# AlonKellner/hifi-gan

Measured on NVIDIA B200. Metric: V1 audio samples/sec, higher is better.
Workload: dtype bf16

## Files before the change

hifi-gan_b200/_lib.py:

```python
from __future__ import annotations

import ctypes
import hashlib
import os
import shutil
import subprocess
import threading
import time
from ctypes import POINTER, byref, c_char_p, c_double, c_float, c_int, c_int64, c_void_p

_HERE = os.path.dirname(os.path.abspath(__file__))
CSRC = os.path.join(_HERE, "csrc")
LIB_PATH = os.path.join(_HERE, "libhifigan_b200.so")
SOURCES = ["hg_api.cu", "hg_conv1d_tc.cu", "hg_resblock_pair.cu", "hg_disc.cu", "hg_prep.cu", "hg_mel.cu",
           "hg_wgrad.cu", "hg_train.cu", "hg_batched.cu"]
NVCC_FLAGS = ["-gencode", "arch=compute_100a,code=sm_100a", "-O3", "-lineinfo", "-std=c++17",
              "-Xcompiler", "-fPIC", "-shared"]

_lock = threading.Lock()
_lib = None


class HgError(RuntimeError):
    pass


HASH_PATH = os.path.join(_HERE, "libhifigan_b200.srchash")
_LOCK_PATH = os.path.join(_HERE, ".build.lock")


def _source_hash() -> str:
    h = hashlib.sha256(" ".join(NVCC_FLAGS).encode())
    deps = sorted(os.path.join(CSRC, f) for f in os.listdir(CSRC) if f.endswith((".cu", ".cuh", ".h")))
    deps.append(os.path.join(os.path.dirname(_HERE), "include", "hifigan_b200.h"))
    for d in deps:
        if os.path.isfile(d):
            h.update(os.path.basename(d).encode())
            with open(d, "rb") as f:
                h.update(f.read())
    return h.hexdigest()


def _stale() -> bool:
    if not os.path.exists(LIB_PATH) or not os.path.exists(HASH_PATH):
        return True
    with open(HASH_PATH) as f:
        return f.read().strip() != _source_hash()


def build(force: bool = False, verbose: bool = False) -> str:
    if not force and not _stale():
        return LIB_PATH
    nvcc = shutil.which("nvcc") or "/usr/local/cuda/bin/nvcc"
    if not os.path.exists(nvcc):
        raise HgError("nvcc not found: cannot build libhifigan_b200.so")
    deadline = time.time() + 900
    while True:
        try:
            fd = os.open(_LOCK_PATH, os.O_CREAT | os.O_EXCL | os.O_WRONLY)
            os.close(fd)
            break
        except FileExistsError:
            if time.time() > deadline or time.time() - os.path.getmtime(_LOCK_PATH) > 900:
                try:
                    os.unlink(_LOCK_PATH)
                except FileNotFoundError:
                    pass
            time.sleep(0.5)
    try:
        if not force and not _stale():
            return LIB_PATH
        tmp = LIB_PATH + f".tmp{os.getpid()}"
        cmd = [nvcc] + NVCC_FLAGS + ["-o", tmp] + [os.path.join(CSRC, s) for s in SOURCES]
        if verbose:
            cmd.insert(1, "-Xptxas=-v")
        res = subprocess.run(cmd, capture_output=True, text=True)
        if res.returncode != 0:
            if os.path.exists(tmp):
                os.unlink(tmp)
            raise HgError("nvcc failed:\n" + res.stdout + res.stderr)
        if verbose:
            print(res.stderr)
        os.replace(tmp, LIB_PATH)
        with open(HASH_PATH + ".tmp", "w") as f:
            f.write(_source_hash())
        os.replace(HASH_PATH + ".tmp", HASH_PATH)
    finally:
        try:
            os.unlink(_LOCK_PATH)
        except FileNotFoundError:
            pass
    return LIB_PATH


_SIGNATURES = {
    "hg_version": (c_char_p, []),
    "hg_last_error": (c_char_p, []),
    "hg_abi_version": (c_int, []),
    "hg_launch_count": (c_int64, []),
    "hg_timestamp": (c_int, [c_void_p, c_void_p]),
    "hg_pack_conv1d_weight": (c_int, [c_void_p, c_void_p, c_int, c_int, c_int, c_int, c_void_p, c_void_p]),
    "hg_convtr1d_geometry": (c_int, [c_int, c_int, c_int, POINTER(c_int), POINTER(c_int)]),
    "hg_pack_convtr1d_weight": (c_int, [c_void_p, c_void_p, c_int, c_int, c_int, c_int, c_int, c_void_p, c_void_p]),
    "hg_conv1d_fwd": (c_int, [c_void_p, c_void_p, c_void_p, c_int, c_int, c_int, c_int, c_int, c_int, c_int,
                              c_void_p, c_void_p, c_void_p, c_float, c_void_p, c_void_p, c_float, c_void_p, c_int,
                              c_void_p]),
    "hg_conv1d_tap_order": (c_int, [c_int, c_int, c_int, POINTER(c_int)]),
    "hg_conv1d_general_fwd": (c_int, [c_void_p, c_void_p, c_void_p, c_int, c_int, c_int, c_int, c_int, c_int, c_int,
                                      c_int, c_int, c_int, c_void_p, c_float, c_void_p, c_int, c_int, c_void_p]),
    "hg_disc_first_conv_fwd": (c_int, [c_void_p, c_void_p, c_void_p, c_int, c_int, c_int, c_int, c_int, c_int, c_int,
                                       c_int, c_void_p, c_float, c_void_p]),
    "hg_disc_last_conv_fwd": (c_int, [c_void_p, c_void_p, c_void_p, c_int, c_int, c_int, c_int, c_int, c_void_p,
                                      c_void_p]),
    "hg_avgpool_4_2_2_fwd": (c_int, [c_void_p, c_int, c_int, c_void_p, c_void_p]),
    "hg_disc_export_fmap": (c_int, [c_void_p, c_int, c_int, c_int, c_int, c_int, c_void_p, c_void_p]),
    "hg_disc_import_fmap": (c_int, [c_void_p, c_int, c_int, c_int, c_int, c_int, c_void_p, c_void_p]),
    "hg_prep_job_size": (c_int, []),
    "hg_prep_batched": (c_int, [c_void_p, c_void_p, c_int, c_int, c_int, c_void_p]),
    "hg_resblock_pair_supported": (c_int, [c_int, c_int, c_int]),
    "hg_resblock_single_supported": (c_int, [c_int, c_int, c_int]),
    "hg_resblock_pair_fwd": (c_int, [c_void_p, c_void_p, c_void_p, c_void_p, c_void_p, c_int, c_int, c_int, c_int,
                                     c_int, c_float, c_void_p, c_void_p, c_float, c_void_p, c_void_p, c_float,
                                     c_void_p, c_int, c_void_p]),
    "hg_float_to_int16": (c_int, [c_void_p, ctypes.c_longlong, c_float, c_void_p, c_void_p]),
    "hg_loss_sum": (c_int, [c_void_p, c_void_p, ctypes.c_longlong, c_int, c_float, c_void_p, c_void_p]),
    "hg_segment_gather": (c_int, [c_void_p, c_void_p, c_void_p, c_int, c_int, c_void_p, c_void_p]),
    "hg_ncl_to_nlc": (c_int, [c_void_p, c_int, c_int, c_int, c_int, c_void_p, c_void_p, c_float, c_void_p]),
    "hg_nlc_to_ncl": (c_int, [c_void_p, c_int, c_int, c_int, c_void_p, c_void_p]),
    "hg_conv_post_tanh_fwd": (c_int, [c_void_p, c_void_p, c_void_p, c_int, c_int, c_int, c_int, c_void_p, c_void_p]),
    "hg_mel_plan_create": (c_int, [POINTER(c_void_p), c_int, c_int, c_int, c_int, c_int, c_double, c_double, c_void_p]),
    "hg_mel_plan_destroy": (c_int, [c_void_p]),
    "hg_mel_num_frames": (c_int, [c_void_p, c_int]),
    "hg_mel_fwd": (c_int, [c_void_p, c_void_p, c_int, c_int, c_void_p, c_void_p, c_void_p]),
    "hg_mel_bwd": (c_int, [c_void_p, c_void_p, c_void_p, c_int, c_int, c_void_p, c_void_p]),
    "hg_mel_emulate_host": (c_int, [c_void_p, c_void_p, c_int, c_int, c_void_p]),
    "hg_mel_bwd_emulate_host": (c_int, [c_void_p, c_void_p, c_void_p, c_int, c_int, c_void_p]),
    "hg_pack_dgrad_weight": (c_int, [c_void_p, c_int, c_int, c_int, c_void_p, c_void_p]),
    "hg_conv1d_dgrad": (c_int, [c_void_p, c_void_p] + [c_int] * 12 + [c_void_p, c_float, c_void_p, c_void_p, c_float,
                                c_void_p, c_void_p, c_void_p, c_float, c_void_p, c_int, c_int, c_int, c_int,
                                c_void_p, c_void_p, c_void_p, c_void_p, c_int, c_void_p]),
    "hg_conv1d_wgrad": (c_int, [c_void_p, c_void_p] + [c_int] * 11 + [c_void_p, c_int, c_void_p]),
    "hg_unpack_wgrad_conv": (c_int, [c_void_p] + [c_int] * 7 + [POINTER(c_int), c_void_p, c_void_p]),
    "hg_wgrad_finish_conv": (c_int, [c_void_p] + [c_int] * 7 + [POINTER(c_int), c_void_p, c_void_p, c_int, c_void_p,
                                                                  c_void_p, c_void_p]),
    "hg_wgrad_finish_convtr": (c_int, [c_void_p] + [c_int] * 7 + [c_void_p, c_void_p, c_int, c_void_p, c_void_p,
                                                                    c_void_p]),
    "hg_weight_norm_bwd": (c_int, [c_void_p, c_void_p, c_void_p, c_int, c_int, c_int, c_void_p, c_void_p, c_void_p]),
    "hg_fold_weight_norm": (c_int, [c_void_p, c_void_p, c_int, c_int, c_void_p, c_void_p]),
    "hg_pack_disc_weight": (c_int, [c_void_p] + [c_int] * 7 + [c_void_p, c_void_p, c_void_p]),
    "hg_spectral_norm_fwd": (c_int, [c_void_p, c_void_p, c_void_p, c_int, c_int, c_int, c_void_p, c_void_p, c_void_p,
                                     c_void_p, c_void_p, c_void_p]),
    "hg_spectral_norm_bwd": (c_int, [c_void_p, c_void_p, c_void_p, c_void_p, c_void_p, c_int, c_int, c_int, c_void_p,
                                     c_void_p, c_void_p]),
    "hg_colsum_bf16": (c_int, [c_void_p, c_int, c_int, c_int, c_int, c_int, c_void_p, c_void_p]),
    "hg_conv_post_tanh_bwd": (c_int, [c_void_p, c_void_p, c_void_p, c_void_p, c_int, c_int, c_int, c_int, c_float,
                                      c_float, c_void_p, c_void_p, c_void_p, c_void_p, c_void_p, c_void_p, c_void_p,
                                      c_void_p]),
    "hg_disc_last_conv_bwd": (c_int, [c_void_p, c_void_p, c_void_p, c_int, c_int, c_int, c_int, c_int, c_float,
                                      c_void_p, c_float, c_void_p, c_void_p, c_void_p, c_void_p, c_void_p, c_void_p]),
    "hg_disc_first_conv_bwd": (c_int, [c_void_p, c_void_p, c_void_p] + [c_int] * 8 + [c_void_p] * 4),
    "hg_avgpool_4_2_2_bwd": (c_int, [c_void_p, c_int, c_int, c_void_p, c_void_p]),
    "hg_loss_grad": (c_int, [c_void_p, c_void_p, ctypes.c_longlong, c_int, c_float, c_float, c_float, c_void_p,
                             c_void_p, c_void_p]),
    "hg_adamw_step": (c_int, [c_void_p, c_void_p, c_void_p, c_void_p, ctypes.c_longlong, c_float, c_float, c_float,
                              c_float, c_float, c_int, c_void_p, c_void_p, c_float, c_void_p]),
}

EXPORTED_SYMBOLS = tuple(_SIGNATURES)


def lib() -> ctypes.CDLL:
    global _lib
    if _lib is not None:
        return _lib
    with _lock:
        if _lib is None:
            if _stale():
                build()
            handle = ctypes.CDLL(LIB_PATH)
            for name, (res, args) in _SIGNATURES.items():
                fn = getattr(handle, name)
                fn.restype = res
                fn.argtypes = args
            if handle.hg_abi_version() != 3:
                raise HgError("libhifigan_b200.so ABI mismatch")
            _lib = handle
    return _lib


def check(rc: int, what: str = "") -> None:
    if rc != 0:
        msg = lib().hg_last_error().decode("utf-8", "replace")
        raise HgError(f"{what or 'hifigan_b200'} failed (code {rc}): {msg}")


def launch_count() -> int:
    return int(lib().hg_launch_count())
```

hifi-gan_b200/csrc/hg_common.cuh:

```cuda
#pragma once

#include <cuda_runtime.h>
#include <cuda_bf16.h>
#include <cuda.h>
#include <stdint.h>
#include <stdio.h>

#define HG_OK 0
#define HG_ERR_INVALID (-1)
#define HG_ERR_CUDA (-2)
#define HG_ERR_UNSUPPORTED (-3)
#define HG_ERR_DRIVER (-4)

void hg_set_error(const char* fmt, ...);

#define HG_CHECK_CUDA(expr)                                                        \
  do {                                                                             \
    cudaError_t _e = (expr);                                                       \
    if (_e != cudaSuccess) {                                                       \
      hg_set_error("%s:%d: %s -> %s", __FILE__, __LINE__, #expr,                   \
                   cudaGetErrorString(_e));                                        \
      return HG_ERR_CUDA;                                                          \
    }                                                                              \
  } while (0)

#define HG_REQUIRE(cond, ...)                                                      \
  do {                                                                             \
    if (!(cond)) {                                                                 \
      hg_set_error(__VA_ARGS__);                                                   \
      return HG_ERR_INVALID;                                                       \
    }                                                                              \
  } while (0)

namespace hg {

#ifndef HG_SPIN_LIMIT
#define HG_SPIN_LIMIT (1u << 28)
#endif

__device__ __forceinline__ uint32_t smem_u32(const void* p) {
  return static_cast<uint32_t>(__cvta_generic_to_shared(p));
}

__device__ __forceinline__ bool elect_one() {
  uint32_t pred = 0;
  asm volatile(
      "{\n\t"
      ".reg .pred P;\n\t"
      "elect.sync _|P, 0xffffffff;\n\t"
      "selp.b32 %0, 1, 0, P;\n\t"
      "}\n"
      : "=r"(pred));
  return pred != 0;
}

__device__ __forceinline__ void mbar_init(uint64_t* bar, uint32_t count) {
  asm volatile("mbarrier.init.shared::cta.b64 [%0], %1;" ::"r"(smem_u32(bar)), "r"(count));
}
__device__ __forceinline__ void fence_mbar_init() {
  asm volatile("fence.mbarrier_init.release.cluster;" ::: "memory");
}
__device__ __forceinline__ void fence_proxy_async_smem() {
  asm volatile("fence.proxy.async.shared::cta;" ::: "memory");
}
__device__ __forceinline__ void mbar_arrive(uint64_t* bar) {
  asm volatile("mbarrier.arrive.shared::cta.b64 _, [%0];" ::"r"(smem_u32(bar)) : "memory");
}
__device__ __forceinline__ void mbar_arrive_expect_tx(uint64_t* bar, uint32_t bytes) {
  asm volatile("mbarrier.arrive.expect_tx.shared::cta.b64 _, [%0], %1;" ::"r"(smem_u32(bar)),
               "r"(bytes)
               : "memory");
}
__device__ __forceinline__ bool mbar_try_wait(uint64_t* bar, uint32_t parity) {
  uint32_t ok;
  asm volatile(
      "{\n\t"
      ".reg .pred P;\n\t"
      "mbarrier.try_wait.parity.shared::cta.b64 P, [%1], %2;\n\t"
      "selp.b32 %0, 1, 0, P;\n\t"
      "}\n"
      : "=r"(ok)
      : "r"(smem_u32(bar)), "r"(parity)
      : "memory");
  return ok != 0;
}
__device__ __forceinline__ void mbar_wait(uint64_t* bar, uint32_t parity) {
  uint32_t spins = 0;
  while (!mbar_try_wait(bar, parity)) {
    if (++spins > HG_SPIN_LIMIT) {
      printf("hg: mbarrier wait timed out (block %d thread %d)\n", (int)blockIdx.x, (int)threadIdx.x);
      __trap();
    }
  }
}

__device__ __forceinline__ void tma_prefetch_desc(const CUtensorMap* m) {
  asm volatile("prefetch.tensormap [%0];" ::"l"(reinterpret_cast<uint64_t>(m)) : "memory");
}
__device__ __forceinline__ void tma_load_3d(void* smem_dst, const CUtensorMap* m, uint64_t* bar,
                                            int32_t c0, int32_t c1, int32_t c2) {
  asm volatile(
      "cp.async.bulk.tensor.3d.shared::cluster.global.mbarrier::complete_tx::bytes"
      " [%0], [%1, {%3, %4, %5}], [%2];"
      :
      : "r"(smem_u32(smem_dst)), "l"(reinterpret_cast<uint64_t>(m)), "r"(smem_u32(bar)), "r"(c0),
        "r"(c1), "r"(c2)
      : "memory");
}

__device__ __forceinline__ void tc_fence_before() {
  asm volatile("tcgen05.fence::before_thread_sync;" ::: "memory");
}
__device__ __forceinline__ void tc_fence_after() {
  asm volatile("tcgen05.fence::after_thread_sync;" ::: "memory");
}
__device__ __forceinline__ void tmem_alloc(uint32_t* smem_result, uint32_t ncols) {
  asm volatile("tcgen05.alloc.cta_group::1.sync.aligned.shared::cta.b32 [%0], %1;" ::"r"(
                   smem_u32(smem_result)),
               "r"(ncols)
               : "memory");
  asm volatile("tcgen05.relinquish_alloc_permit.cta_group::1.sync.aligned;" ::: "memory");
}
__device__ __forceinline__ void tmem_dealloc(uint32_t taddr, uint32_t ncols) {
  asm volatile("tcgen05.dealloc.cta_group::1.sync.aligned.b32 %0, %1;" ::"r"(taddr), "r"(ncols)
               : "memory");
}
__device__ __forceinline__ void umma_bf16_ss_lo(uint32_t d_tmem, uint32_t a_lo, uint32_t b_lo,
                                                uint32_t desc_hi, uint32_t idesc, uint32_t accumulate) {
  asm volatile(
      "{\n\t"
      ".reg .pred p;\n\t"
      ".reg .b64 da, db;\n\t"
      "setp.ne.b32 p, %5, 0;\n\t"
      "mov.b64 da, {%1, %3};\n\t"
      "mov.b64 db, {%2, %3};\n\t"
      "tcgen05.mma.cta_group::1.kind::f16 [%0], da, db, %4, p;\n\t"
      "}\n"
      :
      : "r"(d_tmem), "r"(a_lo), "r"(b_lo), "r"(desc_hi), "r"(idesc), "r"(accumulate)
      : "memory");
}
__device__ __forceinline__ uint32_t cluster_ctarank() {
  uint32_t r;
  asm volatile("mov.u32 %0, %%cluster_ctarank;" : "=r"(r));
  return r;
}
__device__ __forceinline__ void cluster_sync_all() {
  asm volatile("barrier.cluster.arrive.release.aligned;" ::: "memory");
  asm volatile("barrier.cluster.wait.acquire.aligned;" ::: "memory");
}
__device__ __forceinline__ void mbar_arrive_remote(uint64_t* bar, uint32_t cta) {
  asm volatile(
      "{\n\t"
      ".reg .b32 remAddr32;\n\t"
      "mapa.shared::cluster.u32 remAddr32, %0, %1;\n\t"
      "mbarrier.arrive.shared::cluster.b64 _, [remAddr32];\n\t"
      "}\n"
      :
      : "r"(smem_u32(bar)), "r"(cta)
      : "memory");
}
__device__ __forceinline__ void tma_load_3d_2sm(void* smem_dst, const CUtensorMap* m, uint64_t* bar,
                                                int32_t c0, int32_t c1, int32_t c2) {
  asm volatile(
      "cp.async.bulk.tensor.3d.cta_group::2.shared::cluster.global.mbarrier::complete_tx::bytes"
      " [%0], [%1, {%3, %4, %5}], [%2];"
      :
      : "r"(smem_u32(smem_dst)), "l"(reinterpret_cast<uint64_t>(m)), "r"(smem_u32(bar) & 0xFEFFFFFFu),
        "r"(c0), "r"(c1), "r"(c2)
      : "memory");
}
__device__ __forceinline__ void tmem_alloc_2sm(uint32_t* smem_result, uint32_t ncols) {
  asm volatile("tcgen05.alloc.cta_group::2.sync.aligned.shared::cta.b32 [%0], %1;" ::"r"(
                   smem_u32(smem_result)),
               "r"(ncols)
               : "memory");
  asm volatile("tcgen05.relinquish_alloc_permit.cta_group::2.sync.aligned;" ::: "memory");
}
__device__ __forceinline__ void tmem_dealloc_2sm(uint32_t taddr, uint32_t ncols) {
  asm volatile("tcgen05.dealloc.cta_group::2.sync.aligned.b32 %0, %1;" ::"r"(taddr), "r"(ncols)
               : "memory");
}
__device__ __forceinline__ void umma_bf16_ss_lo_2sm(uint32_t d_tmem, uint32_t a_lo, uint32_t b_lo,
                                                    uint32_t desc_hi, uint32_t idesc, uint32_t accumulate) {
  asm volatile(
      "{\n\t"
      ".reg .pred p;\n\t"
      ".reg .b64 da, db;\n\t"
      "setp.ne.b32 p, %5, 0;\n\t"
      "mov.b64 da, {%1, %3};\n\t"
      "mov.b64 db, {%2, %3};\n\t"
      "tcgen05.mma.cta_group::2.kind::f16 [%0], da, db, %4, p;\n\t"
      "}\n"
      :
      : "r"(d_tmem), "r"(a_lo), "r"(b_lo), "r"(desc_hi), "r"(idesc), "r"(accumulate)
      : "memory");
}
__device__ __forceinline__ void umma_commit_2sm(uint64_t* bar) {
  asm volatile(
      "tcgen05.commit.cta_group::2.mbarrier::arrive::one.shared::cluster.multicast::cluster.b64 [%0], %1;"
      :
      : "r"(smem_u32(bar)), "h"(static_cast<uint16_t>(3))
      : "memory");
}

__device__ __forceinline__ uint32_t umma_desc_lo(uint32_t saddr) {
  return ((saddr & 0x3FFFFu) >> 4) | (1u << 16);
}
__device__ __forceinline__ uint32_t umma_desc_hi(uint32_t sbo_bytes, uint32_t layout_type) {
  return ((sbo_bytes >> 4) & 0x3FFFu) | (1u << 14) | ((layout_type & 7u) << 29);
}
__device__ __forceinline__ void umma_commit(uint64_t* bar) {
  asm volatile("tcgen05.commit.cta_group::1.mbarrier::arrive::one.shared::cluster.b64 [%0];" ::"r"(
                   smem_u32(bar))
               : "memory");
}
__device__ __forceinline__ void tmem_ld_wait() {
  asm volatile("tcgen05.wait::ld.sync.aligned;" ::: "memory");
}


__host__ __device__ constexpr uint32_t umma_idesc_bf16(uint32_t M, uint32_t N) {
  return (1u << 4) | (1u << 7) | (1u << 10) | ((N >> 3) << 17) | ((M >> 4) << 24);
}

__device__ __forceinline__ float lrelu(float v, float slope) { return v > 0.f ? v : v * slope; }

__device__ __forceinline__ uint32_t pack_bf16x2(float lo, float hi) {
  __nv_bfloat162 h = __floats2bfloat162_rn(lo, hi);
  return *reinterpret_cast<uint32_t*>(&h);
}
__device__ __forceinline__ float2 unpack_bf16x2(uint32_t w) {
  __nv_bfloat162 h = *reinterpret_cast<__nv_bfloat162*>(&w);
  return __bfloat1622float2(h);
}

struct U8 {
  uint32_t v[8];
};

__device__ __forceinline__ U8 ldg256(const void* p) {
  U8 r;
  asm volatile("ld.global.nc.L1::no_allocate.v8.b32 {%0,%1,%2,%3,%4,%5,%6,%7}, [%8];"
               : "=r"(r.v[0]), "=r"(r.v[1]), "=r"(r.v[2]), "=r"(r.v[3]), "=r"(r.v[4]), "=r"(r.v[5]),
                 "=r"(r.v[6]), "=r"(r.v[7])
               : "l"(p));
  return r;
}
__device__ __forceinline__ void stg256(void* p, const U8& r) {
  asm volatile("st.global.v8.b32 [%0], {%1,%2,%3,%4,%5,%6,%7,%8};" ::"l"(p), "r"(r.v[0]),
               "r"(r.v[1]), "r"(r.v[2]), "r"(r.v[3]), "r"(r.v[4]), "r"(r.v[5]), "r"(r.v[6]),
               "r"(r.v[7])
               : "memory");
}
__device__ __forceinline__ void tmem_ld_32x16(uint32_t taddr, uint32_t (&v)[16]) {
  asm volatile(
      "tcgen05.ld.sync.aligned.32x32b.x16.b32 "
      "{%0, %1, %2, %3, %4, %5, %6, %7, %8, %9, %10, %11, %12, %13, %14, %15}, [%16];"
      : "=r"(v[0]), "=r"(v[1]), "=r"(v[2]), "=r"(v[3]), "=r"(v[4]), "=r"(v[5]), "=r"(v[6]),
        "=r"(v[7]), "=r"(v[8]), "=r"(v[9]), "=r"(v[10]), "=r"(v[11]), "=r"(v[12]), "=r"(v[13]),
        "=r"(v[14]), "=r"(v[15])
      : "r"(taddr)
      : "memory");
}
__device__ __forceinline__ void add_bf16x16(float (&v)[16], const U8& r) {
#pragma unroll
  for (int i = 0; i < 8; ++i) {
    const float2 f = unpack_bf16x2(r.v[i]);
    v[2 * i] += f.x;
    v[2 * i + 1] += f.y;
  }
}



template <int N>
__device__ __forceinline__ float warp_colsum(float (&v)[N], int lane, int& col) {
  int off = 16;
  col = 0;
#pragma unroll
  for (int w = N / 2; w >= 1; w >>= 1) {
    const bool hi = (lane & off) != 0;
#pragma unroll
    for (int i = 0; i < w; ++i) {
      const float send = hi ? v[i] : v[i + w];
      const float keep = hi ? v[i + w] : v[i];
      v[i] = keep + __shfl_xor_sync(0xffffffffu, send, off);
    }
    if (hi) col += w;
    off >>= 1;
  }
#pragma unroll
  for (int o = 16; o >= 1; o >>= 1)
    if (o <= off) v[0] += __shfl_xor_sync(0xffffffffu, v[0], o);
  return v[0];
}

struct PerDeviceOnce {
  size_t done[64] = {};
  bool need(size_t want = 1) {
    int d = 0;
    if (cudaGetDevice(&d) != cudaSuccess || d < 0 || d >= 64) return true;
    if (done[d] >= want) return false;
    done[d] = want;
    return true;
  }
};
}

int hg_encode_tmap_bf16_3d(CUtensorMap* out, const void* base, uint64_t d0, uint64_t d1, uint64_t d2,
                           uint64_t stride1_bytes, uint64_t stride2_bytes, uint32_t box0,
                           uint32_t box1, uint32_t box2, int swizzle_bytes);
```

hifi-gan_b200/csrc/hg_conv1d_tc.cu:

```cuda
#include "hg_common.cuh"

#include <atomic>
#include <cstdlib>

extern std::atomic<int64_t> g_hg_launches;

namespace {

constexpr int kTileM = 128;
constexpr int kEpiWarps = 8;
constexpr int kThreads = 64 + kEpiWarps * 32;
constexpr int kMaxStages = 8;
constexpr int kMaxASlots = 4;

constexpr int kMaxBoxes = 4;

struct ConvArgs {
  int batch, t, cin, cout;
  int t_pitch;
  int ktaps, dil, pad_left;
  int nchunks, a_rows;
  int nboxes;
  int box_col[kMaxBoxes];
  int box_row[kMaxBoxes];
  int box_ntaps[kMaxBoxes];
  int box_tap0[kMaxBoxes];
  int tap_step;
  int grouped;
  int tiles_t, tiles_n, num_tiles;
  int a_slots;
  int resident;
  int tps;
  int groups;
  int stages;
  uint32_t a_slot_bytes, w_stage_bytes;
  const float* bias;
  const __nv_bfloat16* res0;
  const __nv_bfloat16* res1;
  const __nv_bfloat16* res2;
  float scale;
  __nv_bfloat16* out_raw;
  __nv_bfloat16* out_act;
  float slope;
  const __nv_bfloat16* mask;
  float mask_slope;
  const __nv_bfloat16* fm_r;
  const __nv_bfloat16* fm_g;
  float fm_coef;
  int group_mod;
  int seq_pitch, seq_valid, seq_mul, seq_div;
  const __nv_bfloat16* pre_add;
  float* colsum[3];
  int colsum_mod;
  const int* item_len;
  int item_mul;
};

__host__ __device__ constexpr bool epi_mask(int k) { return k >= 2; }
__host__ __device__ constexpr bool epi_sums(int k) { return k == 2 || k == 4; }
__host__ __device__ constexpr bool epi_fm(int k) { return k == 3 || k == 4; }
__host__ __device__ constexpr bool epi_pre(int k) { return k == 4; }
__host__ __device__ constexpr bool epi_mrf(int k) { return k >= 2; }
template <int kEpi>
__device__ __forceinline__ void epi_group(const ConvArgs& p, bool valid, bool keep, size_t off, int ch,
                                          const uint32_t (&raw)[16], const hg::U8* r0, const hg::U8* r1,
                                          const hg::U8* r2, float (&v)[16]) {
  if (!valid) {
#pragma unroll
    for (int e = 0; e < 16; ++e) v[e] = 0.f;
    return;
  }
#pragma unroll
  for (int e = 0; e < 16; ++e) v[e] = __uint_as_float(raw[e]);
  if (p.bias) {
#pragma unroll
    for (int q = 0; q < 4; ++q) {
      const float4 bq = __ldg(reinterpret_cast<const float4*>(p.bias + ch + q * 4));
      v[4 * q] += bq.x; v[4 * q + 1] += bq.y; v[4 * q + 2] += bq.z; v[4 * q + 3] += bq.w;
    }
  }
  if (epi_fm(kEpi) && p.fm_g) {
    const hg::U8 fg = hg::ldg256(p.fm_g + off), fr = hg::ldg256(p.fm_r + off);
#pragma unroll
    for (int i = 0; i < 8; ++i) {
      const float2 a = hg::unpack_bf16x2(fg.v[i]), r = hg::unpack_bf16x2(fr.v[i]);
      v[2 * i] += p.fm_coef * ((a.x > r.x) ? 1.f : (a.x < r.x) ? -1.f : 0.f);
      v[2 * i + 1] += p.fm_coef * ((a.y > r.y) ? 1.f : (a.y < r.y) ? -1.f : 0.f);
    }
  }
  if (epi_pre(kEpi) && p.pre_add) hg::add_bf16x16(v, hg::ldg256(p.pre_add + off));
  if (epi_mask(kEpi) && p.mask) {
    const hg::U8 mk = hg::ldg256(p.mask + off);
#pragma unroll
    for (int i = 0; i < 8; ++i) {
      const float2 a = hg::unpack_bf16x2(mk.v[i]);
      if (!(a.x > 0.f)) v[2 * i] *= p.mask_slope;
      if (!(a.y > 0.f)) v[2 * i + 1] *= p.mask_slope;
    }
  }
  if (p.res0) hg::add_bf16x16(v, *r0);
  if (epi_mrf(kEpi) && p.res1) hg::add_bf16x16(v, r1 ? *r1 : hg::ldg256(p.res1 + off));
  if (epi_mrf(kEpi) && p.res2) hg::add_bf16x16(v, r2 ? *r2 : hg::ldg256(p.res2 + off));
  const float sc = keep ? p.scale : 0.f;
#pragma unroll
  for (int e = 0; e < 16; ++e) v[e] *= sc;
  if (p.out_raw) {
    hg::U8 o;
#pragma unroll
    for (int i = 0; i < 8; ++i) o.v[i] = hg::pack_bf16x2(v[2 * i], v[2 * i + 1]);
    hg::stg256(p.out_raw + off, o);
  }
  if (p.out_act) {
    hg::U8 o;
#pragma unroll
    for (int i = 0; i < 8; ++i)
      o.v[i] = hg::pack_bf16x2(hg::lrelu(v[2 * i], p.slope), hg::lrelu(v[2 * i + 1], p.slope));
    hg::stg256(p.out_act + off, o);
  }
}

__device__ __forceinline__ void epi_colsum16(float (&v)[16], int lane, float* csum) {
  int col;
  const float sum = hg::warp_colsum<16>(v, lane, col);
  if (!(lane & 1)) atomicAdd(csum + col, sum);
}

__device__ __forceinline__ void epi_bar_sync() { asm volatile("bar.sync 1, %0;" ::"n"(kEpiWarps * 32) : "memory"); }

template <int NT>
__device__ __forceinline__ void epi_colsum_flush(const ConvArgs& p, float* csum, int nt, int epi_tid) {
  epi_bar_sync();
  for (int c = epi_tid; c < NT; c += kEpiWarps * 32) {
    const float sum = csum[c];
    csum[c] = 0.f;
    const int gc = (nt * NT + c) % p.colsum_mod;
    if (sum != 0.f) {
      atomicAdd(p.colsum[0] + gc, sum);
      if (p.colsum[1]) atomicAdd(p.colsum[1] + gc, sum);
      if (p.colsum[2]) atomicAdd(p.colsum[2] + gc, sum);
    }
  }
  epi_bar_sync();
}

struct Barriers {
  uint64_t a_full[kMaxASlots];
  uint64_t a_empty[kMaxASlots];
  uint64_t w_full[kMaxStages];
  uint64_t w_empty[kMaxStages];
  uint64_t acc_full[2];
  uint64_t acc_empty[2];
  uint32_t tmem_base;
  uint32_t pad;
};

struct TileIter {
  int nt, tt, b, tile;
  int step_n, step_t, step_b;
  int tiles_n, tiles_t;
  __device__ __forceinline__ TileIter(const ConvArgs& p) {
    tiles_n = p.tiles_n; tiles_t = p.tiles_t;
    tile = blockIdx.x;
    nt = tile % tiles_n;
    const int r = tile / tiles_n;
    tt = r % tiles_t; b = r / tiles_t;
    const int g = gridDim.x;
    step_n = g % tiles_n;
    const int gr = g / tiles_n;
    step_t = gr % tiles_t; step_b = gr / tiles_t;
  }
  __device__ __forceinline__ void next() {
    tile += gridDim.x;
    nt += step_n;
    int carry = 0;
    if (nt >= tiles_n) { nt -= tiles_n; carry = 1; }
    tt += step_t + carry;
    carry = 0;
    if (tt >= tiles_t) { tt -= tiles_t; carry = 1; }
    b += step_b + carry;
  }
};

template <int KC, int NT, int kEpi>
__global__ void __launch_bounds__(kThreads, 1)
conv1d_tc_kernel(const __grid_constant__ CUtensorMap tm_x, const __grid_constant__ CUtensorMap tm_w,
                 const ConvArgs p) {
  constexpr uint32_t kRowBytes = KC * 2;
  constexpr uint32_t kLayout = (KC == 64) ? 2u : 4u;
  constexpr uint32_t kSbo = 8 * kRowBytes;
  constexpr uint32_t kTapBytes = NT * kRowBytes;
  constexpr uint32_t kTmemCols = (2 * NT <= 32) ? 32u : (2 * NT <= 64) ? 64u
                                 : (2 * NT <= 128) ? 128u : (2 * NT <= 256) ? 256u : 512u;
  constexpr int kColsPerWarp = NT / 2;
  constexpr int kGroups16 = kColsPerWarp / 16;

  extern __shared__ uint8_t smem_raw[];
  uint8_t* smem = reinterpret_cast<uint8_t*>((reinterpret_cast<uintptr_t>(smem_raw) + 1023) &
                                             ~static_cast<uintptr_t>(1023));
  uint8_t* a_buf = smem;
  uint8_t* w_buf = smem + p.a_slots * p.a_slot_bytes;
  const uint32_t w_total = p.resident ? static_cast<uint32_t>(p.nchunks * p.ktaps) * kTapBytes
                                      : static_cast<uint32_t>(p.stages) * p.w_stage_bytes;
  Barriers* bars = reinterpret_cast<Barriers*>(w_buf + w_total);

  const int warp = threadIdx.x >> 5;
  const int lane = threadIdx.x & 31;

  if (warp == 0 && lane == 0) {
    hg::tma_prefetch_desc(&tm_x);
    hg::tma_prefetch_desc(&tm_w);
  }
  if (warp == 1) {
    if (lane == 0) {
      for (int i = 0; i < kMaxASlots; ++i) {
        hg::mbar_init(&bars->a_full[i], 1);
        hg::mbar_init(&bars->a_empty[i], 1);
      }
      for (int i = 0; i < 2; ++i) {
        hg::mbar_init(&bars->acc_full[i], 1);
        hg::mbar_init(&bars->acc_empty[i], kEpiWarps);
      }
      for (int i = 0; i < kMaxStages; ++i) {
        hg::mbar_init(&bars->w_full[i], 1);
        hg::mbar_init(&bars->w_empty[i], 1);
      }
      hg::fence_mbar_init();
    }
    __syncwarp();
    hg::tmem_alloc(&bars->tmem_base, kTmemCols);
  }
  hg::tc_fence_before();
  __syncthreads();
  hg::tc_fence_after();
  const uint32_t tmem_base = *reinterpret_cast<volatile uint32_t*>(&bars->tmem_base);

  if (warp == 0) {
    if (lane == 0) {
      uint32_t a_slot = 0, a_phase = 0, w_slot = 0, w_phase = 0;
      const uint32_t a_bytes = static_cast<uint32_t>(p.a_rows) * kRowBytes;
      if (p.resident) {
        hg::mbar_arrive_expect_tx(&bars->w_full[0], w_total);
        for (int c = 0; c < p.nchunks; ++c)
          hg::tma_load_3d(w_buf + static_cast<uint32_t>(c * p.ktaps) * kTapBytes, &tm_w,
                          &bars->w_full[0], c * KC, 0, 0);
      }
      for (TileIter it(p); it.tile < p.num_tiles; it.next()) {
        const int nt = it.nt, b = it.b;
        const int t0 = it.tt * kTileM;
        const int chan0 = p.grouped ? (nt % p.group_mod) * p.cin : 0;
        for (int c = 0; c < p.nchunks; ++c) {
          int in_stage = 0;
          for (int bx = 0; bx < p.nboxes; ++bx) {
            const uint32_t slot = a_slot;
            hg::mbar_wait(&bars->a_empty[slot], a_phase ^ 1u);
            hg::mbar_arrive_expect_tx(&bars->a_full[slot], a_bytes);
            hg::tma_load_3d(a_buf + slot * p.a_slot_bytes, &tm_x, &bars->a_full[slot],
                            p.box_col[bx] + chan0 + c * KC, t0 + p.box_row[bx], b);
            if (++a_slot == static_cast<uint32_t>(p.a_slots)) { a_slot = 0; a_phase ^= 1u; }
            if (!p.resident) {
              const int q_end = p.box_tap0[bx] + p.box_ntaps[bx];
              for (int q = p.box_tap0[bx]; q < q_end; ++q) {
                const bool first_of_stage = in_stage == 0;
                if (++in_stage == p.tps) in_stage = 0;
                if (!first_of_stage) continue;
                const uint32_t s = w_slot;
                hg::mbar_wait(&bars->w_empty[s], w_phase ^ 1u);
                hg::mbar_arrive_expect_tx(&bars->w_full[s], static_cast<uint32_t>(p.tps) * kTapBytes);
                hg::tma_load_3d(w_buf + s * p.w_stage_bytes, &tm_w, &bars->w_full[s], c * KC, nt * NT, q);
                if (++w_slot == static_cast<uint32_t>(p.stages)) { w_slot = 0; w_phase ^= 1u; }
              }
            }
          }
        }
      }
    }
    __syncwarp();
  } else if (warp == 1) {
    constexpr uint32_t idesc = hg::umma_idesc_bf16(kTileM, NT);
    constexpr uint32_t kTapLo = kTapBytes >> 4;
    const uint32_t desc_hi = hg::umma_desc_hi(kSbo, kLayout);
    const uint32_t a_tap_step = static_cast<uint32_t>(p.tap_step) * (kRowBytes >> 4);
    const uint32_t w_lo0 = hg::umma_desc_lo(hg::smem_u32(w_buf));
    uint32_t acc_it = 0;
    uint32_t a_slot = 0, a_phase = 0;
    uint32_t w_slot = 0, w_phase = 0;
    if (p.resident) {
      hg::mbar_wait(&bars->w_full[0], 0);
      hg::tc_fence_after();
    }
    const bool leader = hg::elect_one();
    for (int tile = blockIdx.x; tile < p.num_tiles; tile += gridDim.x) {
      const uint32_t acc = acc_it & 1u;
      hg::mbar_wait(&bars->acc_empty[acc], ((acc_it >> 1) & 1u) ^ 1u);
      hg::tc_fence_after();
      const uint32_t d_tmem = tmem_base + acc * NT;
      uint32_t accumulate = 0;
      for (int c = 0; c < p.nchunks; ++c) {
        int in_stage = 0;
        uint32_t w_stage_lo = 0;
        for (int bx = 0; bx < p.nboxes; ++bx) {
          const uint32_t slot = a_slot;
          hg::mbar_wait(&bars->a_full[slot], a_phase);
          hg::tc_fence_after();
          uint32_t a_lo = hg::umma_desc_lo(hg::smem_u32(a_buf + slot * p.a_slot_bytes));
          const int q0 = p.box_tap0[bx], q_end = q0 + p.box_ntaps[bx];
          if (p.resident) {
            if (leader) {
              uint32_t w_lo = w_lo0 + static_cast<uint32_t>(c * p.ktaps + q0) * kTapLo;
              uint32_t acc_flag = accumulate;
              for (int q = q0; q < q_end; ++q) {
#pragma unroll
                for (int kk = 0; kk < KC / 16; ++kk) {
                  hg::umma_bf16_ss_lo(d_tmem, a_lo + kk * 2, w_lo + kk * 2, desc_hi, idesc, acc_flag);
                  acc_flag = 1;
                }
                a_lo += a_tap_step;
                w_lo += kTapLo;
              }
            }
            accumulate = 1;
          } else {
            for (int q = q0; q < q_end; ++q) {
              if (in_stage == 0) {
                hg::mbar_wait(&bars->w_full[w_slot], w_phase);
                hg::tc_fence_after();
                w_stage_lo = w_lo0 + ((w_slot * p.w_stage_bytes) >> 4);
              }
              const bool stage_done = (in_stage == p.tps - 1) || (q == p.ktaps - 1);
              if (leader) {
#pragma unroll
                for (int kk = 0; kk < KC / 16; ++kk) {
                  hg::umma_bf16_ss_lo(d_tmem, a_lo + kk * 2, w_stage_lo + kk * 2, desc_hi, idesc, accumulate);
                  accumulate = 1;
                }
                if (stage_done) hg::umma_commit(&bars->w_empty[w_slot]);
              }
              accumulate = 1;
              a_lo += a_tap_step;
              w_stage_lo += kTapLo;
              if (stage_done) {
                in_stage = 0;
                if (++w_slot == static_cast<uint32_t>(p.stages)) { w_slot = 0; w_phase ^= 1u; }
              } else {
                ++in_stage;
              }
            }
          }
          if (leader) hg::umma_commit(&bars->a_empty[slot]);
          __syncwarp();
          if (++a_slot == static_cast<uint32_t>(p.a_slots)) { a_slot = 0; a_phase ^= 1u; }
        }
      }
      if (leader) hg::umma_commit(&bars->acc_full[acc]);
      __syncwarp();
      ++acc_it;
    }
  } else {
    const int ew = warp - 2;
    const int quarter = warp & 3;
    const int half = ew >> 2;
    const int row = quarter * 32 + lane;
    const int col0 = half * kColsPerWarp;
    uint32_t acc_it = 0;
    float* csum = reinterpret_cast<float*>(bars + 1);
    const int epi_tid = threadIdx.x - 64;
    int cs_nt = -1;
    if (epi_sums(kEpi) && p.colsum[0]) {
      for (int c = epi_tid; c < NT; c += kEpiWarps * 32) csum[c] = 0.f;
      epi_bar_sync();
    }
    for (TileIter it(p); it.tile < p.num_tiles; it.next()) {
      const int nt = it.nt, b = it.b;
      if (epi_sums(kEpi) && p.colsum[0] && nt != cs_nt) {
        if (cs_nt >= 0) epi_colsum_flush<NT>(p, csum, cs_nt, epi_tid);
        cs_nt = nt;
      }
      const int t = it.tt * kTileM + row;
      bool valid = t < p.t;
      if (kEpi >= 1 && p.seq_pitch) valid = valid && ((t % p.seq_pitch) * p.seq_mul + (nt * NT) / p.seq_div < p.seq_valid);
      const bool keep = !p.item_len || t < __ldg(p.item_len + b) * p.item_mul;
      const int ch0 = nt * NT + col0;
      const size_t off = (static_cast<size_t>(b) * p.t_pitch + (valid ? t : 0)) * p.cout + ch0;
      hg::U8 rpre[kGroups16];
      if (p.res0 && valid) {
#pragma unroll
        for (int g = 0; g < kGroups16; ++g) rpre[g] = hg::ldg256(p.res0 + off + g * 16);
      }
      constexpr bool kPreAll = kGroups16 <= 4;
      hg::U8 rpre1[kPreAll ? kGroups16 : 1], rpre2[kPreAll ? kGroups16 : 1];
      if (epi_mrf(kEpi) && kPreAll && valid) {
        if (p.res1) {
#pragma unroll
          for (int g = 0; g < kGroups16; ++g) rpre1[kPreAll ? g : 0] = hg::ldg256(p.res1 + off + g * 16);
        }
        if (p.res2) {
#pragma unroll
          for (int g = 0; g < kGroups16; ++g) rpre2[kPreAll ? g : 0] = hg::ldg256(p.res2 + off + g * 16);
        }
      }
      const uint32_t acc = acc_it & 1u;
      hg::mbar_wait(&bars->acc_full[acc], (acc_it >> 1) & 1u);
      hg::tc_fence_after();
#pragma unroll
      for (int g = 0; g < kGroups16; ++g) {
        uint32_t raw[16];
        const uint32_t taddr = tmem_base + (static_cast<uint32_t>(quarter * 32) << 16) + acc * NT +
                               col0 + g * 16;
        hg::tmem_ld_32x16(taddr, raw);
        hg::tmem_ld_wait();
        float v[16];
        epi_group<kEpi>(p, valid, keep, off + g * 16, ch0 + g * 16, raw, &rpre[g], kPreAll ? &rpre1[kPreAll ? g : 0] : nullptr,
                  kPreAll ? &rpre2[kPreAll ? g : 0] : nullptr, v);
        if (epi_sums(kEpi) && p.colsum[0]) epi_colsum16(v, lane, csum + col0 + g * 16);
      }
      hg::tc_fence_before();
      __syncwarp();
      if (lane == 0) hg::mbar_arrive(&bars->acc_empty[acc]);
      ++acc_it;
    }
    if (epi_sums(kEpi) && p.colsum[0] && cs_nt >= 0) epi_colsum_flush<NT>(p, csum, cs_nt, epi_tid);
  }

  hg::tc_fence_before();
  __syncthreads();
  hg::tc_fence_after();
  if (warp == 1) hg::tmem_dealloc(tmem_base, kTmemCols);
}

struct Barriers2 {
  uint64_t a_full[kMaxASlots];
  uint64_t a_empty[kMaxASlots];
  uint64_t w_full[kMaxStages];
  uint64_t w_empty[kMaxStages];
  uint64_t acc_full[2];
  uint64_t acc_empty[2];
  uint32_t tmem_base;
  uint32_t pad;
};

template <int NT, int kEpi>
__global__ void __cluster_dims__(2, 1, 1) __launch_bounds__(kThreads, 1)
conv1d_tc2_kernel(const __grid_constant__ CUtensorMap tm_x, const __grid_constant__ CUtensorMap tm_w,
                  const ConvArgs p) {
  constexpr int KC = 64;
  constexpr uint32_t kRowBytes = KC * 2;
  constexpr uint32_t kLayout = 2u;
  constexpr uint32_t kSbo = 8 * kRowBytes;
  constexpr uint32_t kTapBytes = (NT / 2) * kRowBytes;
  constexpr uint32_t kTmemCols = (2 * NT <= 256) ? 256u : 512u;
  constexpr int kColsPerWarp = NT / 2;
  constexpr int kGroups16 = kColsPerWarp / 16;

  extern __shared__ uint8_t smem_raw[];
  uint8_t* smem = reinterpret_cast<uint8_t*>((reinterpret_cast<uintptr_t>(smem_raw) + 1023) &
                                             ~static_cast<uintptr_t>(1023));
  uint8_t* a_buf = smem;
  uint8_t* w_buf = smem + p.a_slots * p.a_slot_bytes;
  Barriers2* bars = reinterpret_cast<Barriers2*>(w_buf + static_cast<uint32_t>(p.stages) * p.w_stage_bytes);

  const int warp = threadIdx.x >> 5;
  const int lane = threadIdx.x & 31;
  const uint32_t rank = hg::cluster_ctarank();
  const int n_clusters = gridDim.x >> 1;
  const int cluster_id = blockIdx.x >> 1;
  const int tiles_pt = (p.tiles_t + 1) >> 1;
  const int num_pt = p.batch * tiles_pt * p.tiles_n;

  if (warp == 0 && lane == 0) {
    hg::tma_prefetch_desc(&tm_x);
    hg::tma_prefetch_desc(&tm_w);
  }
  if (warp == 1) {
    if (lane == 0) {
      for (int i = 0; i < kMaxASlots; ++i) {
        hg::mbar_init(&bars->a_full[i], 2);
        hg::mbar_init(&bars->a_empty[i], 1);
      }
      for (int i = 0; i < 2; ++i) {
        hg::mbar_init(&bars->acc_full[i], 1);
        hg::mbar_init(&bars->acc_empty[i], 2 * kEpiWarps);
      }
      for (int i = 0; i < kMaxStages; ++i) {
        hg::mbar_init(&bars->w_full[i], 2);
        hg::mbar_init(&bars->w_empty[i], 1);
      }
      hg::fence_mbar_init();
    }
    __syncwarp();
    hg::tmem_alloc_2sm(&bars->tmem_base, kTmemCols);
  }
  hg::tc_fence_before();
  __syncthreads();
  hg::cluster_sync_all();
  hg::tc_fence_after();
  const uint32_t tmem_base = *reinterpret_cast<volatile uint32_t*>(&bars->tmem_base);

  auto decode = [&](int pt, int& nt, int& ptt, int& b) {
    nt = pt % p.tiles_n;
    const int r = pt / p.tiles_n;
    ptt = r % tiles_pt;
    b = r / tiles_pt;
  };

  if (warp == 0) {
    if (lane == 0) {
      uint32_t a_slot = 0, a_phase = 0, w_slot = 0, w_phase = 0;
      const uint32_t a_bytes = static_cast<uint32_t>(p.a_rows) * kRowBytes;
      const uint32_t w_bytes = static_cast<uint32_t>(p.tps) * kTapBytes;
      for (int pt = cluster_id; pt < num_pt; pt += n_clusters) {
        int nt, ptt, b;
        decode(pt, nt, ptt, b);
        const int t0 = (2 * ptt + static_cast<int>(rank)) * kTileM - p.pad_left;
        for (int c = 0; c < p.nchunks; ++c) {
          hg::mbar_wait(&bars->a_empty[a_slot], a_phase ^ 1u);
          if (rank == 0) hg::mbar_arrive_expect_tx(&bars->a_full[a_slot], 2 * a_bytes);
          else hg::mbar_arrive_remote(&bars->a_full[a_slot], 0);
          hg::tma_load_3d_2sm(a_buf + a_slot * p.a_slot_bytes, &tm_x, &bars->a_full[a_slot], c * KC, t0, b);
          if (++a_slot == static_cast<uint32_t>(p.a_slots)) { a_slot = 0; a_phase ^= 1u; }
          for (int g = 0; g < p.groups; ++g) {
            hg::mbar_wait(&bars->w_empty[w_slot], w_phase ^ 1u);
            if (rank == 0) hg::mbar_arrive_expect_tx(&bars->w_full[w_slot], 2 * w_bytes);
            else hg::mbar_arrive_remote(&bars->w_full[w_slot], 0);
            hg::tma_load_3d_2sm(w_buf + w_slot * p.w_stage_bytes, &tm_w, &bars->w_full[w_slot], c * KC,
                                nt * NT + static_cast<int>(rank) * (NT / 2), g * p.tps);
            if (++w_slot == static_cast<uint32_t>(p.stages)) { w_slot = 0; w_phase ^= 1u; }
          }
        }
      }
    }
    __syncwarp();
  } else if (warp == 1) {
    if (rank == 0) {
      constexpr uint32_t idesc = hg::umma_idesc_bf16(2 * kTileM, NT);
      constexpr uint32_t kTapLo = kTapBytes >> 4;
      const uint32_t desc_hi = hg::umma_desc_hi(kSbo, kLayout);
      const uint32_t a_tap_step = static_cast<uint32_t>(p.tap_step) * (kRowBytes >> 4);
      const uint32_t w_lo0 = hg::umma_desc_lo(hg::smem_u32(w_buf));
      const bool leader = hg::elect_one();
      uint32_t acc_it = 0, a_slot = 0, a_phase = 0, w_slot = 0, w_phase = 0;
      for (int pt = cluster_id; pt < num_pt; pt += n_clusters) {
        const uint32_t acc = acc_it & 1u;
        hg::mbar_wait(&bars->acc_empty[acc], ((acc_it >> 1) & 1u) ^ 1u);
        hg::tc_fence_after();
        const uint32_t d_tmem = tmem_base + acc * NT;
        uint32_t accumulate = 0;
        for (int c = 0; c < p.nchunks; ++c) {
          hg::mbar_wait(&bars->a_full[a_slot], a_phase);
          hg::tc_fence_after();
          uint32_t a_lo = hg::umma_desc_lo(hg::smem_u32(a_buf + a_slot * p.a_slot_bytes));
          int q = 0;
          for (int g = 0; g < p.groups; ++g) {
            hg::mbar_wait(&bars->w_full[w_slot], w_phase);
            hg::tc_fence_after();
            if (leader) {
              uint32_t w_lo = w_lo0 + ((w_slot * p.w_stage_bytes) >> 4);
              const int q_end = min(p.ktaps, q + p.tps);
              for (int j = q; j < q_end; ++j) {
#pragma unroll
                for (int kk = 0; kk < KC / 16; ++kk) {
                  hg::umma_bf16_ss_lo_2sm(d_tmem, a_lo + kk * 2, w_lo + kk * 2, desc_hi, idesc, accumulate);
                  accumulate = 1;
                }
                a_lo += a_tap_step;
                w_lo += kTapLo;
              }
              hg::umma_commit_2sm(&bars->w_empty[w_slot]);
            } else {
              a_lo += a_tap_step * static_cast<uint32_t>(min(p.ktaps, q + p.tps) - q);
            }
            accumulate = 1;
            q += p.tps;
            __syncwarp();
            if (++w_slot == static_cast<uint32_t>(p.stages)) { w_slot = 0; w_phase ^= 1u; }
          }
          if (leader) hg::umma_commit_2sm(&bars->a_empty[a_slot]);
          __syncwarp();
          if (++a_slot == static_cast<uint32_t>(p.a_slots)) { a_slot = 0; a_phase ^= 1u; }
        }
        if (leader) hg::umma_commit_2sm(&bars->acc_full[acc]);
        __syncwarp();
        ++acc_it;
      }
    }
  } else {
    const int ew = warp - 2;
    const int quarter = warp & 3;
    const int half = ew >> 2;
    const int row = quarter * 32 + lane;
    const int col0 = half * kColsPerWarp;
    uint32_t acc_it = 0;
    float* csum = reinterpret_cast<float*>(bars + 1);
    const int epi_tid = threadIdx.x - 64;
    int cs_nt = -1;
    if (epi_sums(kEpi) && p.colsum[0]) {
      for (int c = epi_tid; c < NT; c += kEpiWarps * 32) csum[c] = 0.f;
      epi_bar_sync();
    }
    for (int pt = cluster_id; pt < num_pt; pt += n_clusters) {
      int nt, ptt, b;
      decode(pt, nt, ptt, b);
      if (epi_sums(kEpi) && p.colsum[0] && nt != cs_nt) {
        if (cs_nt >= 0) epi_colsum_flush<NT>(p, csum, cs_nt, epi_tid);
        cs_nt = nt;
      }
      const int t = (2 * ptt + static_cast<int>(rank)) * kTileM + row;
      bool valid = t < p.t;
      if (kEpi >= 1 && p.seq_pitch) valid = valid && ((t % p.seq_pitch) * p.seq_mul + (nt * NT) / p.seq_div < p.seq_valid);
      const bool keep = !p.item_len || t < __ldg(p.item_len + b) * p.item_mul;
      const int ch0 = nt * NT + col0;
      const size_t off = (static_cast<size_t>(b) * p.t_pitch + (valid ? t : 0)) * p.cout + ch0;
      hg::U8 rpre[kGroups16];
      if (p.res0 && valid) {
#pragma unroll
        for (int g = 0; g < kGroups16; ++g) rpre[g] = hg::ldg256(p.res0 + off + g * 16);
      }
      constexpr bool kPreAll = kGroups16 <= 4;
      hg::U8 rpre1[kPreAll ? kGroups16 : 1], rpre2[kPreAll ? kGroups16 : 1];
      if (epi_mrf(kEpi) && kPreAll && valid) {
        if (p.res1) {
#pragma unroll
          for (int g = 0; g < kGroups16; ++g) rpre1[kPreAll ? g : 0] = hg::ldg256(p.res1 + off + g * 16);
        }
        if (p.res2) {
#pragma unroll
          for (int g = 0; g < kGroups16; ++g) rpre2[kPreAll ? g : 0] = hg::ldg256(p.res2 + off + g * 16);
        }
      }
      const uint32_t acc = acc_it & 1u;
      hg::mbar_wait(&bars->acc_full[acc], (acc_it >> 1) & 1u);
      hg::tc_fence_after();
#pragma unroll
      for (int g = 0; g < kGroups16; ++g) {
        uint32_t raw[16];
        const uint32_t taddr = tmem_base + (static_cast<uint32_t>(quarter * 32) << 16) + acc * NT + col0 + g * 16;
        hg::tmem_ld_32x16(taddr, raw);
        hg::tmem_ld_wait();
        float v[16];
        epi_group<kEpi>(p, valid, keep, off + g * 16, ch0 + g * 16, raw, &rpre[g], kPreAll ? &rpre1[kPreAll ? g : 0] : nullptr,
                  kPreAll ? &rpre2[kPreAll ? g : 0] : nullptr, v);
        if (epi_sums(kEpi) && p.colsum[0]) epi_colsum16(v, lane, csum + col0 + g * 16);
      }
      hg::tc_fence_before();
      __syncwarp();
      if (lane == 0) {
        if (rank == 0) hg::mbar_arrive(&bars->acc_empty[acc]);
        else hg::mbar_arrive_remote(&bars->acc_empty[acc], 0);
      }
      ++acc_it;
    }
    if (epi_sums(kEpi) && p.colsum[0] && cs_nt >= 0) epi_colsum_flush<NT>(p, csum, cs_nt, epi_tid);
  }

  hg::tc_fence_before();
  __syncthreads();
  hg::cluster_sync_all();
  hg::tc_fence_after();
  if (warp == 1) hg::tmem_dealloc_2sm(tmem_base, kTmemCols);
}

int g_num_sms = 0;
int g_max_smem = 0;

int device_props() {
  if (g_num_sms) return HG_OK;
  int dev = 0;
  HG_CHECK_CUDA(cudaGetDevice(&dev));
  HG_CHECK_CUDA(cudaDeviceGetAttribute(&g_num_sms, cudaDevAttrMultiProcessorCount, dev));
  HG_CHECK_CUDA(cudaDeviceGetAttribute(&g_max_smem, cudaDevAttrMaxSharedMemoryPerBlockOptin, dev));
  return HG_OK;
}

template <int KC, int NT, int kEpi>
int launch_as(const CUtensorMap& tm_x, const CUtensorMap& tm_w, const ConvArgs& p, size_t smem_bytes,
              int grid, cudaStream_t st) {
  static hg::PerDeviceOnce once;
  if (once.need())
    HG_CHECK_CUDA(cudaFuncSetAttribute(conv1d_tc_kernel<KC, NT, kEpi>,
                                       cudaFuncAttributeMaxDynamicSharedMemorySize, g_max_smem));
  conv1d_tc_kernel<KC, NT, kEpi><<<grid, kThreads, smem_bytes, st>>>(tm_x, tm_w, p);
  HG_CHECK_CUDA(cudaGetLastError());
  return HG_OK;
}

int epi_flavour(const ConvArgs& p) {
  if (p.pre_add || (p.fm_g && p.colsum[0])) return 4;
  if (p.fm_g) return 3;
  if (p.mask || p.colsum[0]) return 2;
  if (p.res1 || p.res2) return 5;
  return p.seq_pitch ? 1 : 0;
}

template <int KC, int NT>
int launch(const CUtensorMap& tm_x, const CUtensorMap& tm_w, const ConvArgs& p, size_t smem_bytes,
           int grid, cudaStream_t st) {
  switch (epi_flavour(p)) {
    case 0: return launch_as<KC, NT, 0>(tm_x, tm_w, p, smem_bytes, grid, st);
    case 1: return launch_as<KC, NT, 1>(tm_x, tm_w, p, smem_bytes, grid, st);
    case 2: return launch_as<KC, NT, 2>(tm_x, tm_w, p, smem_bytes, grid, st);
    case 3: return launch_as<KC, NT, 3>(tm_x, tm_w, p, smem_bytes, grid, st);
    case 5: return launch_as<KC, NT, 5>(tm_x, tm_w, p, smem_bytes, grid, st);
    default: return launch_as<KC, NT, 4>(tm_x, tm_w, p, smem_bytes, grid, st);
  }
}

template <int NT, int kEpi>
int launch2_as(const CUtensorMap& tm_x, const CUtensorMap& tm_w, const ConvArgs& p, size_t smem_bytes, int grid,
               cudaStream_t st) {
  static hg::PerDeviceOnce once;
  if (once.need())
    HG_CHECK_CUDA(cudaFuncSetAttribute(conv1d_tc2_kernel<NT, kEpi>, cudaFuncAttributeMaxDynamicSharedMemorySize,
                                       g_max_smem));
  conv1d_tc2_kernel<NT, kEpi><<<grid, kThreads, smem_bytes, st>>>(tm_x, tm_w, p);
  HG_CHECK_CUDA(cudaGetLastError());
  return HG_OK;
}

template <int NT>
int launch2(const CUtensorMap& tm_x, const CUtensorMap& tm_w, const ConvArgs& p, size_t smem_bytes, int grid,
            cudaStream_t st) {
  switch (epi_flavour(p)) {
    case 0: return launch2_as<NT, 0>(tm_x, tm_w, p, smem_bytes, grid, st);
    case 1: return launch2_as<NT, 1>(tm_x, tm_w, p, smem_bytes, grid, st);
    case 2: return launch2_as<NT, 2>(tm_x, tm_w, p, smem_bytes, grid, st);
    case 3: return launch2_as<NT, 3>(tm_x, tm_w, p, smem_bytes, grid, st);
    case 5: return launch2_as<NT, 5>(tm_x, tm_w, p, smem_bytes, grid, st);
    default: return launch2_as<NT, 4>(tm_x, tm_w, p, smem_bytes, grid, st);
  }
}

int g_use_2cta = -1;

struct TapPlan {
  int nboxes;
  int box_col_mult[kMaxBoxes];
  int box_row[kMaxBoxes], box_ntaps[kMaxBoxes], box_tap0[kMaxBoxes];
  int tap_step, max_ntaps;
  int order[256];
};

int make_tap_plan(int ktaps, int stride, int dilation, int pad_left, TapPlan* tp) {
  if (ktaps < 1 || ktaps > 256 || stride < 1 || stride > kMaxBoxes || dilation < 1) return -1;
  if (stride > 1 && dilation != 1) return -1;
  tp->nboxes = 0;
  tp->max_ntaps = 0;
  if (stride == 1) {
    tp->nboxes = 1;
    tp->box_col_mult[0] = 0; tp->box_row[0] = -pad_left; tp->box_ntaps[0] = ktaps; tp->box_tap0[0] = 0;
    tp->tap_step = dilation; tp->max_ntaps = ktaps;
    for (int j = 0; j < ktaps; ++j) tp->order[j] = j;
    return 0;
  }
  tp->tap_step = 1;
  int q_packed = 0;
  for (int rho = 0; rho < stride; ++rho) {
    int n = 0, qmin = 0;
    for (int j = 0; j < ktaps; ++j) {
      const int e = j - pad_left;
      const int r = ((e % stride) + stride) % stride;
      if (r != rho) continue;
      const int q = (e - r) / stride;
      if (n == 0) qmin = q;
      tp->order[q_packed + n] = j;
      ++n;
    }
    if (!n) continue;
    const int b = tp->nboxes++;
    tp->box_col_mult[b] = rho; tp->box_row[b] = qmin; tp->box_ntaps[b] = n; tp->box_tap0[b] = q_packed;
    q_packed += n;
    if (n > tp->max_ntaps) tp->max_ntaps = n;
  }
  return 0;
}

struct ConvExtra {
  const void* mask = nullptr;
  float mask_slope = 1.f;
  const void* fm_r = nullptr;
  const void* fm_g = nullptr;
  float fm_coef = 0.f;
  int group_mod = 0;
  int t_in_valid = -1;
  int seq_pitch = 0, seq_valid = 0, seq_mul = 1, seq_div = 1 << 30;
  const void* pre_add = nullptr;
  float* colsum[3] = {nullptr, nullptr, nullptr};
  int colsum_mod = 0;
  const int* item_len = nullptr;
  int item_mul = 1;
};

int conv_forward(const void* x, const void* w_packed, const float* bias, int batch, int t_in_rows,
                 int c_total, int t_out, int t_out_rows, int cin_tile, int cout, int n_tile, int grouped, int ktaps,
                 int stride, int dilation, int pad_left, const void* res0, const void* res1,
                 const void* res2, float scale, void* out_raw, void* out_act, float act_slope,
                 void* stream, const ConvExtra& ex = ConvExtra()) {
  HG_REQUIRE(x && w_packed, "conv: null input");
  HG_REQUIRE(out_raw || out_act, "conv: no output requested");
  HG_REQUIRE(batch > 0 && t_out > 0 && t_in_rows > 0, "conv: empty batch/time");
  HG_REQUIRE(cin_tile % 32 == 0 && cin_tile > 0, "conv: cin=%d must be a multiple of 32", cin_tile);
  HG_REQUIRE(cout % 32 == 0 && cout > 0, "conv: cout=%d must be a multiple of 32", cout);
  HG_REQUIRE(n_tile == 32 || n_tile == 64 || n_tile == 128 || n_tile == 256, "conv: bad N tile %d", n_tile);
  HG_REQUIRE(cout % n_tile == 0, "conv: cout %d is not a multiple of the N tile %d", cout, n_tile);
  HG_REQUIRE(t_in_rows % stride == 0, "conv: input rows %d must be a multiple of the stride %d",
             t_in_rows, stride);
  TapPlan tp;
  HG_REQUIRE(make_tap_plan(ktaps, stride, dilation, pad_left, &tp) == 0,
             "conv: unsupported taps/stride/dilation (%d,%d,%d)", ktaps, stride, dilation);
  const int a_rows = kTileM + (tp.max_ntaps - 1) * tp.tap_step;
  HG_REQUIRE(a_rows <= 256, "conv: halo too large for one TMA box (rows=%d > 256)", a_rows);
  int rc = device_props();
  if (rc) return rc;

  const int kc = (cin_tile % 64 == 0) ? 64 : 32;
  ConvArgs p{};
  HG_REQUIRE(t_out_rows >= t_out, "conv: output pitch %d < rows %d", t_out_rows, t_out);
  p.batch = batch; p.t = t_out; p.t_pitch = t_out_rows; p.cin = cin_tile; p.cout = cout;
  p.ktaps = ktaps; p.dil = dilation; p.pad_left = pad_left;
  p.nchunks = cin_tile / kc;
  p.a_rows = a_rows;
  p.nboxes = tp.nboxes;
  for (int b = 0; b < tp.nboxes; ++b) {
    p.box_col[b] = tp.box_col_mult[b] * c_total;
    p.box_row[b] = tp.box_row[b];
    p.box_ntaps[b] = tp.box_ntaps[b];
    p.box_tap0[b] = tp.box_tap0[b];
  }
  p.tap_step = tp.tap_step;
  p.grouped = grouped;
  p.tiles_t = (t_out + kTileM - 1) / kTileM;
  p.tiles_n = cout / n_tile;
  p.num_tiles = batch * p.tiles_t * p.tiles_n;
  p.a_slot_bytes = (static_cast<uint32_t>(a_rows) * kc * 2 + 1023u) & ~1023u;
  const uint32_t tap_bytes = static_cast<uint32_t>(n_tile) * kc * 2;
  const int colsum_bytes = ex.colsum[0] ? 1024 : 0;
  const int budget = g_max_smem - 1024  - static_cast<int>(sizeof(Barriers)) - colsum_bytes;

  const long long w_all = static_cast<long long>(ktaps) * p.nchunks * tap_bytes;
  uint32_t w_bytes_total;
  if (p.tiles_n == 1 && w_all + 2LL * p.a_slot_bytes <= budget && w_all < (1 << 20)) {
    p.resident = 1;
    p.tps = ktaps; p.groups = 1; p.stages = 1;
    p.w_stage_bytes = static_cast<uint32_t>(w_all);
    w_bytes_total = static_cast<uint32_t>(w_all);
  } else {
    p.resident = 0;
    p.tps = tap_bytes >= 32768 ? 1 : static_cast<int>(32768 / tap_bytes);
    if (p.tps > ktaps) p.tps = ktaps;
    p.groups = (ktaps + p.tps - 1) / p.tps;
    p.w_stage_bytes = static_cast<uint32_t>(p.tps) * tap_bytes;
    int stages = (budget - 2 * static_cast<int>(p.a_slot_bytes)) / static_cast<int>(p.w_stage_bytes);
    if (stages > 4) stages = 4;
    HG_REQUIRE(stages >= 2, "conv: not enough shared memory for the weight ring");
    p.stages = stages;
    w_bytes_total = static_cast<uint32_t>(stages) * p.w_stage_bytes;
  }
  if (g_use_2cta < 0) g_use_2cta = getenv("HG_DISABLE_2CTA") ? 0 : 1;
  const bool pair = g_use_2cta && !p.resident && stride == 1 && !grouped && kc == 64 && n_tile >= 128 &&
                    (g_num_sms % 2 == 0) && batch * p.tiles_t * p.tiles_n >= g_num_sms;
  if (pair) {
    const uint32_t half_tap = tap_bytes / 2;
    p.tps = half_tap >= 32768 ? 1 : static_cast<int>(32768 / half_tap);
    if (p.tps > ktaps) p.tps = ktaps;
    p.groups = (ktaps + p.tps - 1) / p.tps;
    p.w_stage_bytes = static_cast<uint32_t>(p.tps) * half_tap;
    int stages = (budget - 2 * static_cast<int>(p.a_slot_bytes)) / static_cast<int>(p.w_stage_bytes);
    if (stages > 4) stages = 4;
    HG_REQUIRE(stages >= 2, "conv: not enough shared memory for the weight ring");
    p.stages = stages;
    w_bytes_total = static_cast<uint32_t>(stages) * p.w_stage_bytes;
  }
  int a_slots = (budget - static_cast<int>(w_bytes_total)) / static_cast<int>(p.a_slot_bytes);
  if (a_slots > kMaxASlots) a_slots = kMaxASlots;
  HG_REQUIRE(a_slots >= 2, "conv: not enough shared memory for the activation ring");
  p.a_slots = a_slots;

  p.bias = bias;
  p.res0 = static_cast<const __nv_bfloat16*>(res0);
  p.res1 = static_cast<const __nv_bfloat16*>(res1);
  p.res2 = static_cast<const __nv_bfloat16*>(res2);
  p.scale = scale;
  p.out_raw = static_cast<__nv_bfloat16*>(out_raw);
  p.out_act = static_cast<__nv_bfloat16*>(out_act);
  p.slope = act_slope;
  p.mask = static_cast<const __nv_bfloat16*>(ex.mask);
  p.mask_slope = ex.mask_slope;
  p.fm_r = static_cast<const __nv_bfloat16*>(ex.fm_r);
  p.fm_g = static_cast<const __nv_bfloat16*>(ex.fm_g);
  p.fm_coef = ex.fm_coef;
  p.group_mod = ex.group_mod > 0 ? ex.group_mod : p.tiles_n;
  p.seq_pitch = ex.seq_pitch; p.seq_valid = ex.seq_valid; p.seq_mul = ex.seq_mul;
  p.pre_add = static_cast<const __nv_bfloat16*>(ex.pre_add);
  for (int i = 0; i < 3; ++i) p.colsum[i] = ex.colsum[i];
  p.colsum_mod = ex.colsum_mod > 0 ? ex.colsum_mod : cout;
  p.item_len = ex.item_len; p.item_mul = ex.item_mul;
  HG_REQUIRE(!ex.colsum[1] || ex.colsum[0], "conv: bias-gradient destinations must be filled from slot 0");
  p.seq_div = ex.seq_div > 0 ? ex.seq_div : (1 << 30);
  HG_REQUIRE(ex.seq_pitch >= 0 && (ex.seq_pitch == 0 || batch == 1), "conv: flat sequences need batch == 1");
  HG_REQUIRE(!p.fm_g || p.fm_r, "conv: fm_g without fm_r");
  HG_REQUIRE(ex.t_in_valid < 0 || (stride == 1 && ex.t_in_valid <= t_in_rows), "conv: bad input bound");
  const int t_in_bound = ex.t_in_valid >= 0 ? ex.t_in_valid : t_in_rows / stride;

  CUtensorMap tm_x, tm_w;
  const int swz = kc * 2;
  rc = hg_encode_tmap_bf16_3d(&tm_x, x, static_cast<uint64_t>(stride) * c_total, t_in_bound, batch,
                              static_cast<uint64_t>(stride) * c_total * 2,
                              static_cast<uint64_t>(t_in_rows) * c_total * 2, kc, a_rows, 1, swz);
  if (rc) return rc;
  rc = hg_encode_tmap_bf16_3d(&tm_w, w_packed, cin_tile, cout, ktaps, static_cast<uint64_t>(cin_tile) * 2,
                              static_cast<uint64_t>(cout) * cin_tile * 2, kc, pair ? n_tile / 2 : n_tile, p.tps,
                              swz);
  if (rc) return rc;

  const size_t smem_bytes = 1024 + static_cast<size_t>(a_slots) * p.a_slot_bytes + w_bytes_total +
                            sizeof(Barriers) + colsum_bytes;
  const int grid = p.num_tiles < g_num_sms ? p.num_tiles : g_num_sms;
  cudaStream_t st = static_cast<cudaStream_t>(stream);
  if (pair) {
    const size_t smem2 = 1024 + static_cast<size_t>(a_slots) * p.a_slot_bytes + w_bytes_total + sizeof(Barriers2) +
                         colsum_bytes;
    const int grid2 = g_num_sms;
    rc = (n_tile == 256) ? launch2<256>(tm_x, tm_w, p, smem2, grid2, st)
                         : launch2<128>(tm_x, tm_w, p, smem2, grid2, st);
    if (rc) return rc;
    g_hg_launches.fetch_add(1, std::memory_order_relaxed);
    return HG_OK;
  }
#define HG_LAUNCH(KC_, NT_) rc = launch<KC_, NT_>(tm_x, tm_w, p, smem_bytes, grid, st)
  if (kc == 64) {
    if (n_tile == 256) HG_LAUNCH(64, 256);
    else if (n_tile == 128) HG_LAUNCH(64, 128);
    else if (n_tile == 64) HG_LAUNCH(64, 64);
    else HG_LAUNCH(64, 32);
  } else {
    if (n_tile == 256) HG_LAUNCH(32, 256);
    else if (n_tile == 128) HG_LAUNCH(32, 128);
    else if (n_tile == 64) HG_LAUNCH(32, 64);
    else HG_LAUNCH(32, 32);
  }
#undef HG_LAUNCH
  if (rc) return rc;
  g_hg_launches.fetch_add(1, std::memory_order_relaxed);
  return HG_OK;
}

}

extern "C" int hg_conv1d_fwd(const void* x, const void* w_packed, const float* bias, int batch, int t,
                             int cin, int cout, int ktaps, int dilation, int pad_left,
                             const void* res0, const void* res1, const void* res2, float scale,
                             void* out_raw, void* out_act, float act_slope, const int* item_len, int item_mul,
                             void* stream) {
  HG_REQUIRE(cout > 0 && cout % 32 == 0, "hg_conv1d_fwd: cout=%d must be a multiple of 32", cout);
  HG_REQUIRE(cin > 0 && cin % 32 == 0, "hg_conv1d_fwd: cin=%d must be a multiple of 32", cin);
  HG_REQUIRE(ktaps > 0 && dilation > 0 && 128 + (ktaps - 1) * dilation <= 256,
             "hg_conv1d_fwd: halo too large for one TMA box (taps=%d dilation=%d)", ktaps, dilation);
  const int n_tile = (cout % 256 == 0) ? 256 : (cout % 128 == 0) ? 128 : (cout % 64 == 0) ? 64 : 32;
  ConvExtra ex;
  ex.item_len = item_len; ex.item_mul = item_mul > 0 ? item_mul : 1;
  return conv_forward(x, w_packed, bias, batch, t, cin, t, t, cin, cout, n_tile, 0, ktaps, 1, dilation, pad_left,
                      res0, res1, res2, scale, out_raw, out_act, act_slope, stream, ex);
}

extern "C" int hg_conv1d_tap_order(int ktaps, int stride, int pad_left, int* host_order) {
  TapPlan tp;
  HG_REQUIRE(host_order && make_tap_plan(ktaps, stride, 1, pad_left, &tp) == 0,
             "hg_conv1d_tap_order: unsupported (taps=%d stride=%d)", ktaps, stride);
  for (int q = 0; q < ktaps; ++q) host_order[q] = tp.order[q];
  return HG_OK;
}

extern "C" int hg_conv1d_general_fwd(const void* x, const void* w_packed, const float* bias, int batch,
                                     int t_in_rows, int c_total, int t_out, int t_out_rows, int groups,
                                     int cout, int ktaps,
                                     int stride, int pad_left, void* out_act, float act_slope,
                                     void* out_raw, int seq_pitch, int seq_valid, void* stream) {
  HG_REQUIRE(groups >= 1 && c_total % groups == 0 && cout % groups == 0, "hg_conv1d_general_fwd: bad groups");
  const int cin_tile = c_total / groups, n_tile_g = cout / groups;
  ConvExtra ex;
  ex.seq_pitch = seq_pitch; ex.seq_valid = seq_valid;
  if (groups == 1) {
    const int n_tile = (cout % 256 == 0) ? 256 : (cout % 128 == 0) ? 128 : (cout % 64 == 0) ? 64 : 32;
    return conv_forward(x, w_packed, bias, batch, t_in_rows, c_total, t_out, t_out_rows, c_total, cout, n_tile, 0,
                        ktaps,
                        stride, 1, pad_left, nullptr, nullptr, nullptr, 1.f, out_raw, out_act, act_slope,
                        stream, ex);
  }
  return conv_forward(x, w_packed, bias, batch, t_in_rows, c_total, t_out, t_out_rows, cin_tile, cout, n_tile_g, 1,
                      ktaps,
                      stride, 1, pad_left, nullptr, nullptr, nullptr, 1.f, out_raw, out_act, act_slope,
                      stream, ex);
}

extern "C" int hg_conv1d_dgrad(const void* dy, const void* w_packed, int batch, int t_dy_valid, int t_dy_rows,
                               int c_dy_total, int t_out, int t_out_rows, int groups, int n_tile, int cout, int ktaps,
                               int dilation, int pad_left, const void* mask_src, float mask_slope,
                               const void* fm_r, const void* fm_g, float fm_coef, const void* res0, const void* res1,
                               const void* res2, float scale, void* out, int seq_pitch, int seq_valid, int seq_mul,
                               int seq_div, const void* pre_add, float* bias_grad0, float* bias_grad1,
                               float* bias_grad2, int bias_mod, void* stream) {
  HG_REQUIRE(groups >= 1 && c_dy_total % groups == 0, "hg_conv1d_dgrad: bad groups");
  HG_REQUIRE(ktaps > 0 && dilation > 0 && 128 + (ktaps - 1) * dilation <= 256,
             "hg_conv1d_dgrad: halo too large for one TMA box (taps=%d dilation=%d)", ktaps, dilation);
  ConvExtra ex;
  ex.mask = mask_src; ex.mask_slope = mask_slope;
  ex.fm_r = fm_r; ex.fm_g = fm_g; ex.fm_coef = fm_coef;
  ex.t_in_valid = t_dy_valid;
  ex.seq_pitch = seq_pitch; ex.seq_valid = seq_valid; ex.seq_mul = seq_mul > 0 ? seq_mul : 1; ex.seq_div = seq_div;
  ex.pre_add = pre_add;
  ex.colsum[0] = bias_grad0; ex.colsum[1] = bias_grad1; ex.colsum[2] = bias_grad2; ex.colsum_mod = bias_mod;
  const int cin_tile = c_dy_total / groups;
  if (groups == 1) {
    if (n_tile <= 0) n_tile = (cout % 256 == 0) ? 256 : (cout % 128 == 0) ? 128 : (cout % 64 == 0) ? 64 : 32;
    return conv_forward(dy, w_packed, nullptr, batch, t_dy_rows, c_dy_total, t_out, t_out_rows, cin_tile, cout,
                        n_tile, 0, ktaps, 1, dilation, pad_left, res0, res1, res2, scale, out, nullptr, 1.f,
                        stream, ex);
  }
  HG_REQUIRE(n_tile > 0, "hg_conv1d_dgrad: grouped layers need an explicit N tile");
  ex.group_mod = groups;
  return conv_forward(dy, w_packed, nullptr, batch, t_dy_rows, c_dy_total, t_out, t_out_rows, cin_tile, cout,
                      n_tile, 1, ktaps, 1, dilation, pad_left, res0, res1, res2, scale, out, nullptr, 1.f,
                      stream, ex);
}
```

hifi-gan_b200/csrc/hg_resblock_pair.cu:

```cuda
#include "hg_common.cuh"

#include <atomic>

#include "../../include/hifigan_b200.h"

extern std::atomic<int64_t> g_hg_launches;

namespace {

constexpr int kM = 128;
constexpr int kXformWarps = 4;
__host__ __device__ constexpr int epi_halves(int c) { return c == 64 ? 2 : 1; }
__host__ __device__ constexpr int pair_threads(int c) { return 64 + (kXformWarps + 8 * epi_halves(c)) * 32; }
constexpr int kMaxXSlots = 4;

struct PairArgs {
  int batch, t, c;
  int ktaps, dil1;
  int single;
  int subs;
  int r_out;
  int pad1, pad2;
  int a_rows;
  int x_boxes, x_box_rows;
  int tiles_t, num_tiles;
  int x_slots;
  uint32_t x_slot_bytes, t1_slot_bytes, w_bytes;
  const __nv_bfloat16* x;
  const float* b1;
  const float* b2;
  const __nv_bfloat16* res1;
  const __nv_bfloat16* res2;
  float scale, in_slope, out_slope;
  __nv_bfloat16* out_raw;
  __nv_bfloat16* out_act;
  const int* item_len;
  int item_mul;
};

struct PairBarriers {
  uint64_t x_full[kMaxXSlots], x_ready[kMaxXSlots], x_empty[kMaxXSlots];
  uint64_t w_full;
  uint64_t acc1_full[2], acc1_empty[2], t1_full[2], t1_empty[2], acc2_full[2], acc2_empty[2];
  uint32_t tmem_base;
  uint32_t pad;
  __align__(16) float b1[64];
  __align__(16) float b2[64];
};

__device__ __forceinline__ uint32_t lrelu_bf16x2(uint32_t w, __nv_bfloat162 slope2) {
  __nv_bfloat162 v = *reinterpret_cast<__nv_bfloat162*>(&w);
  v = __hmax2(v, __hmul2(v, slope2));
  return *reinterpret_cast<uint32_t*>(&v);
}

template <int C, bool kSingle, bool kMrf>
__global__ void __launch_bounds__(pair_threads(C), 1)
resblock_pair_kernel(const __grid_constant__ CUtensorMap tm_x, const __grid_constant__ CUtensorMap tm_w1,
                     const __grid_constant__ CUtensorMap tm_w2, const PairArgs p) {
  constexpr uint32_t kRowBytes = C * 2;
  constexpr uint32_t kLayout = (C == 64) ? 2u : 4u;
  constexpr uint32_t kSbo = 8 * kRowBytes;
  constexpr uint32_t kTapBytes = C * kRowBytes;
  constexpr int kChunksPerRow = kRowBytes / 16;
  constexpr int kHalves = epi_halves(C);
  constexpr int kRoleWarps = 4 * kHalves;
  constexpr int kThreads = pair_threads(C);

  extern __shared__ uint8_t smem_raw[];
  uint8_t* smem = reinterpret_cast<uint8_t*>((reinterpret_cast<uintptr_t>(smem_raw) + 1023) &
                                             ~static_cast<uintptr_t>(1023));
  uint8_t* x_buf = smem;
  uint8_t* t1_buf = x_buf + p.x_slots * p.x_slot_bytes;
  uint8_t* w1_buf = t1_buf + 2 * p.t1_slot_bytes;
  uint8_t* w2_buf = w1_buf + p.w_bytes;
  PairBarriers* bars = reinterpret_cast<PairBarriers*>(w1_buf + (kSingle ? 1 : 2) * p.w_bytes);

  const int warp = threadIdx.x >> 5;
  const int lane = threadIdx.x & 31;
  const int S = p.subs;
  const uint32_t acc_cols = static_cast<uint32_t>(S) * C;
  const uint32_t tmem_cols = 4 * acc_cols <= 128 ? 128u : 4 * acc_cols <= 256 ? 256u : 512u;

  if (warp == 0 && lane == 0) {
    hg::tma_prefetch_desc(&tm_x);
    hg::tma_prefetch_desc(&tm_w1);
    hg::tma_prefetch_desc(&tm_w2);
  }
  if (warp == 1) {
    if (lane == 0) {
      for (int i = 0; i < kMaxXSlots; ++i) {
        hg::mbar_init(&bars->x_full[i], 1);
        hg::mbar_init(&bars->x_ready[i], kXformWarps);
        hg::mbar_init(&bars->x_empty[i], 1);
      }
      hg::mbar_init(&bars->w_full, 1);
      for (int i = 0; i < 2; ++i) {
        hg::mbar_init(&bars->acc1_full[i], 1);
        hg::mbar_init(&bars->acc1_empty[i], kRoleWarps);
        hg::mbar_init(&bars->t1_full[i], kRoleWarps);
        hg::mbar_init(&bars->t1_empty[i], 1);
        hg::mbar_init(&bars->acc2_full[i], 1);
        hg::mbar_init(&bars->acc2_empty[i], kRoleWarps);
      }
      hg::fence_mbar_init();
    }
    __syncwarp();
    hg::tmem_alloc(&bars->tmem_base, tmem_cols);
  }
  if (threadIdx.x < C) {
    bars->b1[threadIdx.x] = p.b1[threadIdx.x];
    bars->b2[threadIdx.x] = p.b2[threadIdx.x];
  }
  for (uint32_t i = threadIdx.x * 16; i < 2 * p.t1_slot_bytes; i += kThreads * 16)
    *reinterpret_cast<uint4*>(t1_buf + i) = make_uint4(0, 0, 0, 0);
  hg::fence_proxy_async_smem();
  hg::tc_fence_before();
  __syncthreads();
  hg::tc_fence_after();
  const uint32_t tmem_base = *reinterpret_cast<volatile uint32_t*>(&bars->tmem_base);
  const int n_local = (p.num_tiles - static_cast<int>(blockIdx.x) + static_cast<int>(gridDim.x) - 1) /
                      static_cast<int>(gridDim.x);

  if (warp == 0) {
    if (lane == 0) {
      hg::mbar_arrive_expect_tx(&bars->w_full, (kSingle ? 1 : 2) * p.w_bytes);
      hg::tma_load_3d(w1_buf, &tm_w1, &bars->w_full, 0, 0, 0);
      if (!kSingle) hg::tma_load_3d(w2_buf, &tm_w2, &bars->w_full, 0, 0, 0);
      const uint32_t box_bytes = static_cast<uint32_t>(p.x_box_rows) * kRowBytes;
      int tt = blockIdx.x % p.tiles_t, b = blockIdx.x / p.tiles_t;
      const int tt_step = gridDim.x % p.tiles_t, b_step = gridDim.x / p.tiles_t;
      uint32_t slot = 0, phase = 0;
      for (int i = 0; i < n_local; ++i) {
        hg::mbar_wait(&bars->x_empty[slot], phase ^ 1u);
        hg::mbar_arrive_expect_tx(&bars->x_full[slot], box_bytes * p.x_boxes);
        for (int bx = 0; bx < p.x_boxes; ++bx)
          hg::tma_load_3d(x_buf + slot * p.x_slot_bytes + bx * box_bytes, &tm_x, &bars->x_full[slot], 0,
                          tt * p.r_out - p.pad2 - p.pad1 + bx * p.x_box_rows, b);
        if (++slot == static_cast<uint32_t>(p.x_slots)) { slot = 0; phase ^= 1u; }
        tt += tt_step; b += b_step;
        if (tt >= p.tiles_t) { tt -= p.tiles_t; ++b; }
      }
    }
    __syncwarp();
  } else if (warp == 1) {
    constexpr uint32_t idesc = hg::umma_idesc_bf16(kM, C);
    constexpr uint32_t kTapLo = kTapBytes >> 4;
    const uint32_t desc_hi = hg::umma_desc_hi(kSbo, kLayout);
    const uint32_t w1_lo = hg::umma_desc_lo(hg::smem_u32(w1_buf));
    const uint32_t w2_lo = hg::umma_desc_lo(hg::smem_u32(w2_buf));
    const uint32_t x_tap_step = static_cast<uint32_t>(p.dil1) * (kRowBytes >> 4);
    hg::mbar_wait(&bars->w_full, 0);
    hg::tc_fence_after();
    auto issue = [&](uint32_t d, uint32_t a_lo, uint32_t w_lo, uint32_t a_step) {
      uint32_t accumulate = 0;
      for (int j = 0; j < p.ktaps; ++j) {
#pragma unroll
        for (int kk = 0; kk < C / 16; ++kk) {
          hg::umma_bf16_ss_lo(d, a_lo + kk * 2, w_lo + kk * 2, desc_hi, idesc, accumulate);
          accumulate = 1;
        }
        a_lo += a_step;
        w_lo += kTapLo;
      }
    };
    uint32_t x_slot = 0, x_phase = 0;
    auto conv1 = [&](int i) {
      const uint32_t slot = x_slot, a = i & 1u, ph = (i >> 1) & 1u;
      hg::mbar_wait(&bars->x_ready[slot], x_phase);
      if (++x_slot == static_cast<uint32_t>(p.x_slots)) { x_slot = 0; x_phase ^= 1u; }
      hg::mbar_wait(&bars->acc1_empty[a], ph ^ 1u);
      hg::tc_fence_after();
      if (hg::elect_one()) {
        const uint32_t x_lo = hg::umma_desc_lo(hg::smem_u32(x_buf + slot * p.x_slot_bytes));
        for (int m = 0; m < S; ++m)
          issue(tmem_base + a * acc_cols + m * C, x_lo + m * (kM * (kRowBytes >> 4)), w1_lo, x_tap_step);
        hg::umma_commit(&bars->x_empty[slot]);
        hg::umma_commit(&bars->acc1_full[a]);
      }
      __syncwarp();
    };
    auto conv2 = [&](int i) {
      const uint32_t a = i & 1u, ph = (i >> 1) & 1u;
      hg::mbar_wait(&bars->t1_full[a], ph);
      hg::mbar_wait(&bars->acc2_empty[a], ph ^ 1u);
      hg::tc_fence_after();
      if (hg::elect_one()) {
        const uint32_t t_lo = hg::umma_desc_lo(hg::smem_u32(t1_buf + a * p.t1_slot_bytes));
        for (int m = 0; m < S; ++m)
          issue(tmem_base + 2 * acc_cols + a * acc_cols + m * C, t_lo + m * (kM * (kRowBytes >> 4)), w2_lo,
                kRowBytes >> 4);
        hg::umma_commit(&bars->t1_empty[a]);
        hg::umma_commit(&bars->acc2_full[a]);
      }
      __syncwarp();
    };
    if (kSingle) {
      for (int i = 0; i < n_local; ++i) conv1(i);
    } else {
      if (n_local > 0) conv1(0);
      for (int i = 0; i < n_local; ++i) {
        if (i + 1 < n_local) conv1(i + 1);
        conv2(i);
      }
    }
  } else if (warp < 2 + kXformWarps) {
    const int tid = (warp - 2) * 32 + lane;
    const __nv_bfloat162 slope2 = __float2bfloat162_rn(p.in_slope);
    const int n_chunks = p.a_rows * kChunksPerRow;
    uint32_t slot = 0, phase = 0;
    for (int i = 0; i < n_local; ++i) {
      hg::mbar_wait(&bars->x_full[slot], phase);
      uint4* xs = reinterpret_cast<uint4*>(x_buf + slot * p.x_slot_bytes);
      for (int q = tid; q < n_chunks; q += kXformWarps * 32) {
        uint4 v = xs[q];
        v.x = lrelu_bf16x2(v.x, slope2); v.y = lrelu_bf16x2(v.y, slope2);
        v.z = lrelu_bf16x2(v.z, slope2); v.w = lrelu_bf16x2(v.w, slope2);
        xs[q] = v;
      }
      hg::fence_proxy_async_smem();
      __syncwarp();
      if (lane == 0) hg::mbar_arrive(&bars->x_ready[slot]);
      if (++slot == static_cast<uint32_t>(p.x_slots)) { slot = 0; phase ^= 1u; }
    }
  } else {
    const int ew = warp - (2 + kXformWarps);
    const int quarter = warp & 3;
    const int half = (ew >> 2) % kHalves;
    const int row = quarter * 32 + lane;
    const uint32_t lane_base = static_cast<uint32_t>(quarter * 32) << 16;
    constexpr int kG = C / (16 * kHalves);
    const int col0 = half * (C / kHalves);

    if (ew < kRoleWarps) {
      const float* bias = bars->b1;
      const uint32_t swz = (C == 64) ? (row & 7) : ((row >> 1) & 3);
      int tt = blockIdx.x % p.tiles_t;
      int bb = blockIdx.x / p.tiles_t;
      const int tt_step = gridDim.x % p.tiles_t, b_step = gridDim.x / p.tiles_t;
      for (int i = 0; i < (kSingle ? 0 : n_local); ++i) {
        const uint32_t a = i & 1u, ph = (i >> 1) & 1u;
        hg::mbar_wait(&bars->acc1_full[a], ph);
        hg::mbar_wait(&bars->t1_empty[a], ph ^ 1u);
        hg::tc_fence_after();
        const int t_item = (kMrf && p.item_len) ? min(p.t, __ldg(p.item_len + bb) * p.item_mul) : p.t;
        for (int m = 0; m < S; ++m) {
          const int grow = m * kM + row;
          const int time = tt * p.r_out - p.pad2 + grow;
          const bool inside = time >= 0 && time < t_item;
          uint8_t* trow = t1_buf + a * p.t1_slot_bytes + static_cast<uint32_t>(grow) * kRowBytes;
#pragma unroll
          for (int g = 0; g < kG; ++g) {
            uint32_t raw[16];
            hg::tmem_ld_32x16(tmem_base + lane_base + a * acc_cols + m * C + col0 + g * 16, raw);
            hg::tmem_ld_wait();
            if (g == kG - 1 && m == S - 1) {
              hg::tc_fence_before();
              __syncwarp();
              if (lane == 0) hg::mbar_arrive(&bars->acc1_empty[a]);
            }
            uint32_t o[8];
#pragma unroll
            for (int q = 0; q < 4; ++q) {
              const float4 bq = *reinterpret_cast<const float4*>(bias + col0 + g * 16 + 4 * q);
              const float v0 = hg::lrelu(__uint_as_float(raw[4 * q]) + bq.x, p.in_slope);
              const float v1 = hg::lrelu(__uint_as_float(raw[4 * q + 1]) + bq.y, p.in_slope);
              const float v2 = hg::lrelu(__uint_as_float(raw[4 * q + 2]) + bq.z, p.in_slope);
              const float v3 = hg::lrelu(__uint_as_float(raw[4 * q + 3]) + bq.w, p.in_slope);
              o[2 * q] = inside ? hg::pack_bf16x2(v0, v1) : 0u;
              o[2 * q + 1] = inside ? hg::pack_bf16x2(v2, v3) : 0u;
            }
            const uint32_t chunk = (col0 >> 3) + g * 2;
            *reinterpret_cast<uint4*>(trow + ((chunk ^ swz) << 4)) = make_uint4(o[0], o[1], o[2], o[3]);
            *reinterpret_cast<uint4*>(trow + (((chunk + 1) ^ swz) << 4)) = make_uint4(o[4], o[5], o[6], o[7]);
          }
        }
        hg::fence_proxy_async_smem();
        __syncwarp();
        if (lane == 0) hg::mbar_arrive(&bars->t1_full[a]);
        tt += tt_step; bb += b_step;
        if (tt >= p.tiles_t) { tt -= p.tiles_t; ++bb; }
      }
    } else {
      const float* bias = kSingle ? bars->b1 : bars->b2;
      uint64_t* full_bar = kSingle ? bars->acc1_full : bars->acc2_full;
      uint64_t* empty_bar = kSingle ? bars->acc1_empty : bars->acc2_empty;
      const uint32_t acc_base = kSingle ? 0u : 2 * acc_cols;
      int n_tt = blockIdx.x % p.tiles_t, n_b = blockIdx.x / p.tiles_t, n_m = 0;
      const int tt_step = gridDim.x % p.tiles_t, b_step = gridDim.x / p.tiles_t;
      auto next_unit_off = [&](bool& valid, bool& keep) -> size_t {
        const int grow = n_m * kM + row;
        const int time = n_tt * p.r_out + grow;
        valid = grow < p.r_out && time < p.t;
        keep = !kMrf || !p.item_len || time < __ldg(p.item_len + n_b) * p.item_mul;
        const size_t o = (static_cast<size_t>(n_b) * p.t + (valid ? time : 0)) * C + col0;
        if (++n_m == S) {
          n_m = 0;
          n_tt += tt_step; n_b += b_step;
          if (n_tt >= p.tiles_t) { n_tt -= p.tiles_t; ++n_b; }
        }
        return o;
      };
      hg::U8 rcur[kG], rnext[kG];
      bool valid = false, valid_next = false, keep = true, keep_next = true;
      size_t off = 0, off_next = 0;
      const int n_units = n_local * S;
      if (n_units > 0) {
        off_next = next_unit_off(valid_next, keep_next);
        if (valid_next) {
#pragma unroll
          for (int g = 0; g < kG; ++g) rnext[g] = hg::ldg256(p.x + off_next + g * 16);
        }
      }
      int i = 0, m = 0;
      for (int u = 0; u < n_units; ++u) {
        const uint32_t a = i & 1u, ph = (i >> 1) & 1u;
        off = off_next; valid = valid_next; keep = keep_next;
#pragma unroll
        for (int g = 0; g < kG; ++g) rcur[g] = rnext[g];
        if (u + 1 < n_units) {
          off_next = next_unit_off(valid_next, keep_next);
          if (valid_next) {
#pragma unroll
            for (int g = 0; g < kG; ++g) rnext[g] = hg::ldg256(p.x + off_next + g * 16);
          }
        }
        constexpr bool kPreRes = kMrf && (C == 32);
        hg::U8 r1[kPreRes ? kG : 1], r2[kPreRes ? kG : 1];
        if (kPreRes && valid && p.res1) {
#pragma unroll
          for (int g = 0; g < kG; ++g) r1[kPreRes ? g : 0] = hg::ldg256(p.res1 + off + g * 16);
        }
        if (kPreRes && valid && p.res2) {
#pragma unroll
          for (int g = 0; g < kG; ++g) r2[kPreRes ? g : 0] = hg::ldg256(p.res2 + off + g * 16);
        }
        if (m == 0) {
          hg::mbar_wait(&full_bar[a], ph);
          hg::tc_fence_after();
        }
#pragma unroll
        for (int g = 0; g < kG; ++g) {
          uint32_t raw[16];
          hg::tmem_ld_32x16(tmem_base + lane_base + acc_base + a * acc_cols + m * C + col0 + g * 16, raw);
          hg::tmem_ld_wait();
          if (g == kG - 1 && m == S - 1) {
            hg::tc_fence_before();
            __syncwarp();
            if (lane == 0) hg::mbar_arrive(&empty_bar[a]);
          }
          if (valid) {
            float v[16];
#pragma unroll
            for (int q = 0; q < 4; ++q) {
              const float4 bq = *reinterpret_cast<const float4*>(bias + col0 + g * 16 + 4 * q);
              v[4 * q] = __uint_as_float(raw[4 * q]) + bq.x;
              v[4 * q + 1] = __uint_as_float(raw[4 * q + 1]) + bq.y;
              v[4 * q + 2] = __uint_as_float(raw[4 * q + 2]) + bq.z;
              v[4 * q + 3] = __uint_as_float(raw[4 * q + 3]) + bq.w;
            }
            hg::add_bf16x16(v, rcur[g]);
            if (kMrf && p.res1) hg::add_bf16x16(v, kPreRes ? r1[kPreRes ? g : 0] : hg::ldg256(p.res1 + off + g * 16));
            if (kMrf && p.res2) hg::add_bf16x16(v, kPreRes ? r2[kPreRes ? g : 0] : hg::ldg256(p.res2 + off + g * 16));
            if (kMrf) {
              const float sc = keep ? p.scale : 0.f;
#pragma unroll
              for (int e = 0; e < 16; ++e) v[e] *= sc;
            }
            if (p.out_raw) {
              hg::U8 o;
#pragma unroll
              for (int q = 0; q < 8; ++q) o.v[q] = hg::pack_bf16x2(v[2 * q], v[2 * q + 1]);
              hg::stg256(p.out_raw + off + g * 16, o);
            }
            if (kMrf && p.out_act) {
              hg::U8 o;
#pragma unroll
              for (int q = 0; q < 8; ++q)
                o.v[q] = hg::pack_bf16x2(hg::lrelu(v[2 * q], p.out_slope), hg::lrelu(v[2 * q + 1], p.out_slope));
              hg::stg256(p.out_act + off + g * 16, o);
            }
          }
        }
        if (++m == S) { m = 0; ++i; }
      }
    }
  }

  hg::tc_fence_before();
  __syncthreads();
  hg::tc_fence_after();
  if (warp == 1) hg::tmem_dealloc(tmem_base, tmem_cols);
}

int g_sms = 0, g_smem = 0;

template <int C, bool kSingle, bool kMrf>
int launch_pair_as(const CUtensorMap& tx, const CUtensorMap& tw1, const CUtensorMap& tw2, const PairArgs& p,
                size_t smem_bytes, int grid, cudaStream_t st) {
  static hg::PerDeviceOnce once;
  if (once.need())
    HG_CHECK_CUDA(cudaFuncSetAttribute(resblock_pair_kernel<C, kSingle, kMrf>,
                                       cudaFuncAttributeMaxDynamicSharedMemorySize, g_smem));
  resblock_pair_kernel<C, kSingle, kMrf><<<grid, pair_threads(C), smem_bytes, st>>>(tx, tw1, tw2, p);
  HG_CHECK_CUDA(cudaGetLastError());
  return HG_OK;
}

template <int C, bool kSingle>
int launch_pair(const CUtensorMap& tx, const CUtensorMap& tw1, const CUtensorMap& tw2, const PairArgs& p,
                size_t smem_bytes, int grid, cudaStream_t st) {
  const bool mrf = p.res1 || p.res2 || p.out_act || p.item_len || p.scale != 1.f;
  return mrf ? launch_pair_as<C, kSingle, true>(tx, tw1, tw2, p, smem_bytes, grid, st)
             : launch_pair_as<C, kSingle, false>(tx, tw1, tw2, p, smem_bytes, grid, st);
}

size_t pair_smem_bytes(int c, int ktaps, int dil1, int subs, int x_slots, int single, PairArgs* out) {
  const uint32_t row = static_cast<uint32_t>(c) * 2;
  const uint32_t a_rows = subs * kM + (ktaps - 1) * dil1;
  const uint32_t boxes = (a_rows + 255) / 256;
  const uint32_t box_rows = ((a_rows + boxes - 1) / boxes + 15) & ~15u;
  const uint32_t x_slot = (boxes * box_rows * row + 1023u) & ~1023u;
  const uint32_t t1_slot = single ? 0u : ((subs * kM + ktaps - 1) * row + 1023u) & ~1023u;
  const uint32_t w_bytes = static_cast<uint32_t>(ktaps) * c * row;
  if (box_rows > 256) return ~static_cast<size_t>(0);
  if (out) {
    out->subs = subs; out->a_rows = a_rows; out->x_boxes = boxes; out->x_box_rows = box_rows;
    out->x_slot_bytes = x_slot; out->t1_slot_bytes = t1_slot; out->w_bytes = w_bytes;
  }
  return 1024 + static_cast<size_t>(x_slots) * x_slot + 2 * static_cast<size_t>(t1_slot) +
         (single ? 1 : 2) * static_cast<size_t>(w_bytes) + sizeof(PairBarriers);
}

int pick_subs(int c, int ktaps, int dil1, int single) {
  for (int subs = 512 / (4 * c); subs >= 1; subs >>= 1)
    if (pair_smem_bytes(c, ktaps, dil1, subs, 2, single, nullptr) <= static_cast<size_t>(g_smem)) return subs;
  return 0;
}

}

extern "C" int hg_resblock_pair_supported(int c, int ktaps, int dil1) {
  if (!(c == 32 || c == 64) || ktaps < 1 || !(ktaps & 1) || dil1 < 1) return 0;
  if (kM + (ktaps - 1) * dil1 > 256 || ktaps > 65) return 0;
  if (!g_smem) {
    int dev = 0;
    if (cudaGetDevice(&dev) != cudaSuccess) return 0;
    cudaDeviceGetAttribute(&g_sms, cudaDevAttrMultiProcessorCount, dev);
    cudaDeviceGetAttribute(&g_smem, cudaDevAttrMaxSharedMemoryPerBlockOptin, dev);
  }
  return pick_subs(c, ktaps, dil1, 0) > 0 ? 1 : 0;
}

extern "C" int hg_resblock_single_supported(int c, int ktaps, int dil1) {
  if (!hg_resblock_pair_supported(c, 1, 1) && !g_smem) return 0;
  if (!(c == 32 || c == 64) || ktaps < 1 || !(ktaps & 1) || dil1 < 1 || ktaps > 65) return 0;
  return pick_subs(c, ktaps, dil1, 1) > 0 ? 1 : 0;
}

extern "C" int hg_resblock_pair_fwd(const void* x, const void* w1_packed, const float* b1,
                                    const void* w2_packed, const float* b2, int batch, int t, int c,
                                    int ktaps, int dil1, float in_slope, const void* res1,
                                    const void* res2, float scale, void* out_raw, void* out_act,
                                    float out_slope, const int* item_len, int item_mul, void* stream) {
  const int single = w2_packed == nullptr;
  HG_REQUIRE(x && w1_packed && b1 && (single || b2), "hg_resblock_pair_fwd: null input");
  HG_REQUIRE(out_raw || out_act, "hg_resblock_pair_fwd: no output requested");
  HG_REQUIRE(batch > 0 && t > 0, "hg_resblock_pair_fwd: empty batch/time");
  HG_REQUIRE(hg_resblock_pair_supported(c, ktaps, dil1) || (single && hg_resblock_single_supported(c, ktaps, dil1)),
             "hg_resblock_pair_fwd: unsupported shape c=%d k=%d d=%d (use hg_conv1d_fwd)", c, ktaps, dil1);
  PairArgs p{};
  p.batch = batch; p.t = t; p.c = c; p.ktaps = ktaps; p.dil1 = dil1;
  const int subs = pick_subs(c, ktaps, dil1, single);
  p.single = single;
  p.r_out = single ? subs * kM : subs * kM + 1 - ktaps;
  p.pad1 = (ktaps - 1) * dil1 / 2;
  p.pad2 = single ? 0 : (ktaps - 1) / 2;
  p.tiles_t = (t + p.r_out - 1) / p.r_out;
  p.num_tiles = batch * p.tiles_t;
  int slots = kMaxXSlots;
  while (slots > 2 && pair_smem_bytes(c, ktaps, dil1, subs, slots, single, nullptr) > static_cast<size_t>(g_smem)) --slots;
  p.x_slots = slots;
  const size_t smem_bytes = pair_smem_bytes(c, ktaps, dil1, subs, slots, single, &p);
  p.x = static_cast<const __nv_bfloat16*>(x);
  p.b1 = b1; p.b2 = single ? b1 : b2;
  p.res1 = static_cast<const __nv_bfloat16*>(res1);
  p.res2 = static_cast<const __nv_bfloat16*>(res2);
  p.scale = scale; p.in_slope = in_slope; p.out_slope = out_slope;
  p.out_raw = static_cast<__nv_bfloat16*>(out_raw);
  p.out_act = static_cast<__nv_bfloat16*>(out_act);
  p.item_len = item_len; p.item_mul = item_mul > 0 ? item_mul : 1;

  CUtensorMap tx, tw1, tw2;
  const int swz = c * 2;
  int rc = hg_encode_tmap_bf16_3d(&tx, x, c, t, batch, static_cast<uint64_t>(c) * 2,
                                  static_cast<uint64_t>(t) * c * 2, c, p.x_box_rows, 1, swz);
  if (rc) return rc;
  rc = hg_encode_tmap_bf16_3d(&tw1, w1_packed, c, c, ktaps, static_cast<uint64_t>(c) * 2,
                              static_cast<uint64_t>(c) * c * 2, c, c, ktaps, swz);
  if (rc) return rc;
  rc = hg_encode_tmap_bf16_3d(&tw2, single ? w1_packed : w2_packed, c, c, ktaps, static_cast<uint64_t>(c) * 2,
                              static_cast<uint64_t>(c) * c * 2, c, c, ktaps, swz);
  if (rc) return rc;
  const int grid = p.num_tiles < g_sms ? p.num_tiles : g_sms;
  cudaStream_t st = static_cast<cudaStream_t>(stream);
  if (single)
    rc = (c == 64) ? launch_pair<64, true>(tx, tw1, tw2, p, smem_bytes, grid, st)
                   : launch_pair<32, true>(tx, tw1, tw2, p, smem_bytes, grid, st);
  else
    rc = (c == 64) ? launch_pair<64, false>(tx, tw1, tw2, p, smem_bytes, grid, st)
                   : launch_pair<32, false>(tx, tw1, tw2, p, smem_bytes, grid, st);
  if (rc) return rc;
  g_hg_launches.fetch_add(1, std::memory_order_relaxed);
  return HG_OK;
}
```

hifi-gan_b200/models.py:

```python
from __future__ import annotations

import os
import warnings
from ctypes import byref, c_int
from typing import Dict, List, Optional, Tuple

import torch
import torch.nn as nn
from torch.nn import AvgPool1d, Conv1d, Conv2d, ConvTranspose1d
from torch.nn.utils import remove_weight_norm, spectral_norm, weight_norm

from . import _lib
from .utils import get_padding, init_weights

LRELU_SLOPE = 0.1


def _wn(module: nn.Module) -> nn.Module:
    with warnings.catch_warnings():
        warnings.simplefilter("ignore")
        return weight_norm(module)


def _pad_ch(c: int) -> int:
    return 32 if c <= 32 else (c + 63) // 64 * 64


def _stream() -> int:
    return torch.cuda.current_stream().cuda_stream


def _require_cuda(x: torch.Tensor, what: str) -> None:
    if not x.is_cuda:
        raise RuntimeError(f"{what}: hifigan_b200 has no CPU path; move the tensor to a B200 (got {x.device})")


def _wants_grad(x: torch.Tensor, module: nn.Module) -> bool:
    return torch.is_grad_enabled() and (x.requires_grad or any(p.requires_grad for p in module.parameters()))


def _g_v(m: nn.Module) -> Tuple[Optional[torch.Tensor], torch.Tensor]:
    if hasattr(m, "weight_g"):
        return m.weight_g, m.weight_v
    return None, m.weight


class _PackedConv:

    __slots__ = ("module", "kind", "cin", "cout", "cin_p", "cout_p", "taps", "dil", "pad_left", "stride",
                 "w", "bias", "key")

    def __init__(self, module: nn.Module, kind: str, device):
        self.module, self.kind = module, kind
        g, v = _g_v(module)
        if kind == "conv":
            cout, cin, k = v.shape
            self.cin, self.cout, self.taps = cin, cout, k
            self.dil = module.dilation[0]
            self.pad_left = module.padding[0]
            self.stride = 1
            self.cin_p, self.cout_p = _pad_ch(cin), _pad_ch(cout)
            n_rows = self.cout_p
        else:
            cin, cout, k = v.shape
            u, pad = module.stride[0], module.padding[0]
            nshift, smin = c_int(), c_int()
            _lib.check(_lib.lib().hg_convtr1d_geometry(k, u, pad, byref(nshift), byref(smin)))
            if k - 2 * pad != u or module.output_padding[0] != 0:
                raise NotImplementedError("ConvTranspose1d must satisfy out_len == stride * in_len")
            self.cin, self.cout, self.taps = cin, cout, nshift.value
            self.dil, self.pad_left, self.stride = 1, -smin.value, u
            self.cin_p, self.cout_p = _pad_ch(cin), _pad_ch(cout)
            n_rows = u * self.cout_p
        self.w = torch.empty(self.taps, n_rows, self.cin_p, dtype=torch.bfloat16, device=device)
        self.bias = torch.zeros(n_rows, dtype=torch.float32, device=device)
        self.key = None

    def _fingerprint(self):
        g, v = _g_v(self.module)
        b = self.module.bias
        return tuple((t.data_ptr(), t._version) for t in (g, v, b) if t is not None)

    def tensors(self):
        g, v = _g_v(self.module)
        return [t for t in (g, v, self.module.bias) if t is not None]

    def batchable(self) -> bool:
        return all(t.device == self.w.device and t.dtype == torch.float32 and t.is_contiguous() for t in self.tensors())

    def add_pack_job(self, table, phase: str) -> None:
        from . import batched
        m = self.module
        g, v = _g_v(m)
        if self.bias.data_ptr() in [t.data_ptr() for t in self.tensors()]:
            self.bias = torch.zeros(self.w.shape[1], dtype=torch.float32, device=self.w.device)
        if self.kind == "conv":
            table.add(phase, batched.GEN_CONV, self.cout_p, 0, v, g, m.bias, self.w, self.bias,
                      ints=(self.cout, self.cin, self.taps, self.cout_p, self.cin_p))
        else:
            nshift, smin = c_int(), c_int()
            _lib.check(_lib.lib().hg_convtr1d_geometry(m.kernel_size[0], self.stride, m.padding[0], byref(nshift),
                                                       byref(smin)))
            table.add(phase, batched.GEN_CONVTR, self.cin_p, 0, v, g, m.bias, self.w, self.bias,
                      ints=(self.cin, self.cout, m.kernel_size[0], self.cin_p, self.cout_p, self.stride, m.padding[0],
                            nshift.value, smin.value))

    def refresh(self) -> None:
        key = self._fingerprint()
        if key == self.key and not torch.cuda.is_current_stream_capturing():
            return
        L = _lib.lib()
        m = self.module
        g, v = _g_v(m)
        dev = self.w.device
        v = v.detach().to(device=dev, dtype=torch.float32)
        g = None if g is None else g.detach().to(device=dev, dtype=torch.float32).reshape(-1)
        b = m.bias.detach().to(device=dev, dtype=torch.float32) if m.bias is not None else None
        if self.kind == "conv":
            if self.cout_p != self.cout:
                v = torch.cat([v, v.new_zeros(self.cout_p - self.cout, *v.shape[1:])], 0)
                if g is not None:
                    g = torch.cat([g, g.new_zeros(self.cout_p - self.cout)], 0)
            v = v.contiguous()
            _lib.check(L.hg_pack_conv1d_weight(v.data_ptr(), 0 if g is None else g.contiguous().data_ptr(),
                                               self.cout_p, self.cin, self.taps, self.cin_p,
                                               self.w.data_ptr(), _stream()), "hg_pack_conv1d_weight")
            if b is not None and self.cout_p == self.cout and b.is_contiguous():
                self.bias = b
            else:
                self.bias.zero_()
                if b is not None:
                    self.bias[: self.cout].copy_(b)
        else:
            k = m.kernel_size[0]
            if self.cout_p != self.cout or self.cin_p != self.cin:
                vp = v.new_zeros(self.cin_p, self.cout_p, k)
                vp[: self.cin, : self.cout] = v
                v = vp
                if g is not None:
                    g = torch.cat([g, g.new_zeros(self.cin_p - self.cin)], 0)
            v = v.contiguous()
            _lib.check(L.hg_pack_convtr1d_weight(v.data_ptr(), 0 if g is None else g.contiguous().data_ptr(),
                                                 self.cin_p, self.cout_p, k, self.stride, m.padding[0],
                                                 self.w.data_ptr(), _stream()), "hg_pack_convtr1d_weight")
            self.bias.zero_()
            if b is not None:
                self.bias.view(self.stride, self.cout_p)[:, : self.cout].copy_(b.unsqueeze(0).expand(self.stride, -1))
        self.key = key


def _conv(L, x, pc: _PackedConv, batch: int, t: int, *, res=(None, None, None), scale=1.0,
          out_raw=None, out_act=None, slope=LRELU_SLOPE, item=(0, 1)) -> None:
    p = [0 if r is None else r.data_ptr() for r in res]
    _lib.check(L.hg_conv1d_fwd(x.data_ptr(), pc.w.data_ptr(), pc.bias.data_ptr(), batch, t, pc.cin_p,
                               pc.w.shape[1], pc.taps, pc.dil, pc.pad_left, p[0], p[1], p[2], scale,
                               0 if out_raw is None else out_raw.data_ptr(),
                               0 if out_act is None else out_act.data_ptr(), slope, item[0], item[1], _stream()),
               "hg_conv1d_fwd")


def _pair(L, x, pc1: _PackedConv, pc2: _PackedConv, batch: int, t: int, *, res=(None, None), scale=1.0,
          out_raw=None, out_act=None, slope=LRELU_SLOPE, item=(0, 1)) -> None:
    p = [0 if r is None else r.data_ptr() for r in res]
    w2, b2 = (0, 0) if pc2 is None else (pc2.w.data_ptr(), pc2.bias.data_ptr())
    _lib.check(L.hg_resblock_pair_fwd(x.data_ptr(), pc1.w.data_ptr(), pc1.bias.data_ptr(), w2,
                                      b2, batch, t, pc1.cin_p, pc1.taps, pc1.dil, LRELU_SLOPE,
                                      p[0], p[1], scale, 0 if out_raw is None else out_raw.data_ptr(),
                                      0 if out_act is None else out_act.data_ptr(), slope, item[0], item[1], _stream()),
               "hg_resblock_pair_fwd")


_FUSE_PAIRS = True


def _pair_ok(L, pc1: _PackedConv, pc2: _PackedConv) -> bool:
    return bool(_FUSE_PAIRS and pc1.cin_p == pc1.cout_p == pc2.cin_p == pc2.cout_p and pc1.taps == pc2.taps
                and pc2.dil == 1 and L.hg_resblock_pair_supported(pc1.cin_p, pc1.taps, pc1.dil))


def _single_ok(L, pc: _PackedConv) -> bool:
    return bool(_FUSE_PAIRS and pc.cin_p == pc.cout_p and L.hg_resblock_single_supported(pc.cin_p, pc.taps, pc.dil))


def _block_plan(L, block: "nn.Module", packs: List[_PackedConv]) -> List[bool]:
    if not isinstance(block, ResBlock1):
        return [_single_ok(L, pc) for pc in packs]
    return [_pair_ok(L, packs[2 * i], packs[2 * i + 1]) for i in range(len(packs) // 2)]


def _resblock_chain(L, block: "nn.Module", packs: List[_PackedConv], batch: int, t: int, c_p: int,
                    x_raw, x_act, bufs: Dict[str, torch.Tensor], final, item=(0, 1)) -> None:
    two_conv = isinstance(block, ResBlock1)
    fused = _block_plan(L, block, packs)
    steps = len(fused)
    cur_raw, cur_act = x_raw, x_act
    ping = [(bufs["a_raw"], bufs["a_act"]), (bufs["b_raw"], bufs["b_act"])]
    for i in range(steps):
        last = i == steps - 1
        nr, na = ping[i & 1]
        want_act = (not last) and (not fused[i + 1])
        if fused[i]:
            pc1, pc2 = (packs[2 * i], packs[2 * i + 1]) if two_conv else (packs[i], None)
            if last:
                final(dict(pair=(pc1, pc2), x=cur_raw))
            else:
                _pair(L, cur_raw, pc1, pc2, batch, t, out_raw=nr, out_act=na if want_act else None, item=item)
        else:
            if two_conv:
                _conv(L, cur_act, packs[2 * i], batch, t, out_act=bufs["t1"], item=item)
                src, pc = bufs["t1"], packs[2 * i + 1]
            else:
                src, pc = cur_act, packs[i]
            if last:
                final(dict(pc=pc, x=src, res0=cur_raw))
            else:
                _conv(L, src, pc, batch, t, res=(cur_raw, None, None), out_raw=nr,
                      out_act=na if (want_act or not two_conv) else None, item=item)
        cur_raw, cur_act = nr, na


class _StandaloneBlockMixin:

    def _packs(self, device) -> List[_PackedConv]:
        cache = self.__dict__.setdefault("_hg_packs", None)
        convs = self._ordered_convs()
        if cache is None or cache[0].w.device != device:
            cache = [_PackedConv(m, "conv", device) for m in convs]
            self.__dict__["_hg_packs"] = cache
        for pc in cache:
            pc.refresh()
        return cache

    def forward(self, x: torch.Tensor) -> torch.Tensor:
        _require_cuda(x, type(self).__name__)
        if _wants_grad(x, self):
            raise NotImplementedError(f"{type(self).__name__} on its own is an inference surface (call it under "
                                      "torch.no_grad()); it is differentiable as part of Generator")
        L = _lib.lib()
        b, c, t = x.shape
        packs = self._packs(x.device)
        c_p = packs[0].cin_p
        mk = lambda: torch.empty(b, t, c_p, dtype=torch.bfloat16, device=x.device)
        bufs = {k: mk() for k in ("x_raw", "x_act", "t1", "a_raw", "a_act", "b_raw", "b_act", "out")}
        xin = x.contiguous().float()
        _lib.check(L.hg_ncl_to_nlc(xin.data_ptr(), b, c, t, c_p, bufs["x_raw"].data_ptr(),
                                   bufs["x_act"].data_ptr(), LRELU_SLOPE, _stream()), "hg_ncl_to_nlc")

        def final(kw):
            if "pair" in kw:
                _pair(L, kw["x"], *kw["pair"], b, t, out_raw=bufs["out"])
            else:
                _conv(L, kw["x"], kw["pc"], b, t, res=(kw["res0"], None, None), out_raw=bufs["out"])

        _resblock_chain(L, self, packs, b, t, c_p, bufs["x_raw"], bufs["x_act"], bufs, final)
        y = torch.empty(b, c_p, t, dtype=torch.float32, device=x.device)
        _lib.check(L.hg_nlc_to_ncl(bufs["out"].data_ptr(), b, t, c_p, y.data_ptr(), _stream()), "hg_nlc_to_ncl")
        return y[:, :c].contiguous() if c_p != c else y


class ResBlock1(_StandaloneBlockMixin, torch.nn.Module):

    def __init__(self, h, channels, kernel_size=3, dilation=(1, 3, 5)):
        super().__init__()
        self.h = h

        def conv(d):
            return _wn(Conv1d(channels, channels, kernel_size, 1, dilation=d,
                              padding=get_padding(kernel_size, d)))

        self.convs1 = nn.ModuleList([conv(d) for d in dilation[:3]])
        self.convs1.apply(init_weights)
        self.convs2 = nn.ModuleList([conv(1) for _ in dilation[:3]])
        self.convs2.apply(init_weights)

    def _ordered_convs(self):
        out = []
        for c1, c2 in zip(self.convs1, self.convs2):
            out += [c1, c2]
        return out

    def remove_weight_norm(self):
        for m in list(self.convs1) + list(self.convs2):
            remove_weight_norm(m)


class ResBlock2(_StandaloneBlockMixin, torch.nn.Module):

    def __init__(self, h, channels, kernel_size=3, dilation=(1, 3)):
        super().__init__()
        self.h = h
        self.convs = nn.ModuleList([
            _wn(Conv1d(channels, channels, kernel_size, 1, dilation=d, padding=get_padding(kernel_size, d)))
            for d in dilation[:2]])
        self.convs.apply(init_weights)

    def _ordered_convs(self):
        return list(self.convs)

    def remove_weight_norm(self):
        for m in self.convs:
            remove_weight_norm(m)


class _GeneratorEngine:

    def __init__(self, gen: "Generator", device):
        self.gen, self.device = gen, device
        self.pre = _PackedConv(gen.conv_pre, "conv", device)
        self.ups = [_PackedConv(m, "convtr", device) for m in gen.ups]
        self.blocks = [[_PackedConv(m, "conv", device) for m in rb._ordered_convs()] for rb in gen.resblocks]
        post = gen.conv_post
        self.post_cin_p = _pad_ch(post.in_channels)
        self.post_w = torch.zeros(self.post_cin_p, post.kernel_size[0], dtype=torch.float32, device=device)
        self.post_b = torch.zeros(1, dtype=torch.float32, device=device)
        self.post_key = None
        self.table, self.table_ptrs, self.ver_key = None, None, None
        self.ws: Dict[Tuple[int, int], Dict[str, torch.Tensor]] = {}
        self.graphs: Dict[tuple, tuple] = {}
        self.graph_seen = set()

    def packs(self) -> List[_PackedConv]:
        return [self.pre] + self.ups + [pc for blk in self.blocks for pc in blk]

    def _post_tensors(self):
        post = self.gen.conv_post
        g, v = _g_v(post)
        return [t for t in (g, v, post.bias) if t is not None]

    def refresh(self) -> None:
        packs = self.packs()
        tensors = [t for pc in packs for t in pc.tensors()] + self._post_tensors()
        if not all(pc.batchable() for pc in packs) or not all(
                t.device == self.post_w.device and t.dtype == torch.float32 and t.is_contiguous() for t in self._post_tensors()):
            return self._refresh_per_layer()
        ptr_key = tuple(t.data_ptr() for t in tensors)
        ver_key = tuple(t._version for t in tensors)
        if self.table is None or ptr_key != self.table_ptrs:
            from . import batched
            table = batched.JobTable(self.device)
            for pc in packs:
                pc.add_pack_job(table, "pack")
            post = self.gen.conv_post
            g, v = _g_v(post)
            table.add("pack", batched.GEN_POST, 1, 0, v, g, post.bias, self.post_w, self.post_b,
                      ints=(post.in_channels, post.kernel_size[0], self.post_cin_p))
            self.table, self.table_ptrs, self.ver_key = table.finalize(), ptr_key, None
        if ver_key != self.ver_key or torch.cuda.is_current_stream_capturing():
            self.table.launch("pack")
            self.ver_key = ver_key

    def invalidate(self) -> None:
        self.ver_key = None
        self.post_key = None
        for pc in self.packs():
            pc.key = None

    def _refresh_per_layer(self) -> None:
        self.pre.refresh()
        for pc in self.ups:
            pc.refresh()
        for blk in self.blocks:
            for pc in blk:
                pc.refresh()
        post = self.gen.conv_post
        g, v = _g_v(post)
        key = tuple((t.data_ptr(), t._version) for t in (g, v, post.bias) if t is not None)
        if key != self.post_key or torch.cuda.is_current_stream_capturing():
            v32 = v.detach().to(self.device, torch.float32)
            w = v32 if g is None else v32 * (g.detach().to(self.device, torch.float32)
                                             / v32.pow(2).sum(dim=(1, 2), keepdim=True).sqrt())
            self.post_w.zero_()
            self.post_w[: post.in_channels].copy_(w[0])
            self.post_b.copy_(post.bias.detach().to(self.device, torch.float32))
            self.post_key = key

    def workspace(self, batch: int, frames: int) -> Dict[str, torch.Tensor]:
        key = (batch, frames)
        ws = self.ws.get(key)
        if ws is not None:
            return ws
        gen = self.gen
        dev = self.device
        t, sizes = frames, []
        for pc in self.ups:
            t *= pc.stride
            sizes.append(batch * t * pc.cout_p)
        biggest = max(sizes)
        bf = lambda n: torch.empty(n, dtype=torch.bfloat16, device=dev)
        ws = {"mel": bf(batch * frames * self.pre.cin_p), "pre": bf(batch * frames * self.pre.cout_p)}
        names = ["x_raw", "x_act", "t1", "a_raw", "a_act", "b_raw", "b_act", "stage_out"]
        names += [f"r{j}" for j in range(max(1, gen.num_kernels - 1))]
        for n in names:
            ws[n] = bf(biggest)
        ws["y"] = torch.empty(batch, 1, t, dtype=torch.float32, device=dev)
        if len(self.ws) >= 8:
            old = next(iter(self.ws))
            self.ws.pop(old)
            for gk in [k for k in self.graphs if k[:2] == old]:
                self.graphs.pop(gk)
        self.ws[key] = ws
        return ws

    GRAPH_MAX_SAMPLES = 1 << 21

    def forward(self, x: torch.Tensor, time_convs: bool = False, lengths: Optional[torch.Tensor] = None) -> torch.Tensor:
        self.refresh()
        b, c, frames = x.shape
        xin = x.contiguous()
        if xin.dtype != torch.float32:
            xin = xin.float()
        t_out = frames
        for pc in self.ups:
            t_out *= pc.stride
        use_graph = (not time_convs and lengths is None and b * t_out <= self.GRAPH_MAX_SAMPLES
                     and not os.environ.get("HG_DISABLE_GRAPHS") and not torch.cuda.is_current_stream_capturing())
        if not use_graph:
            return self._launch(xin, time_convs, lengths)
        key = (b, frames, _FUSE_PAIRS)
        entry = self.graphs.get(key)
        if entry is None:
            static_in = torch.empty_like(xin)
            static_in.copy_(xin)
            out = self._launch(static_in, False)
            torch.cuda.synchronize()
            if key not in self.graph_seen:
                self.graph_seen.add(key)
                return out
            try:
                graph = torch.cuda.CUDAGraph()
                with torch.cuda.graph(graph):
                    out = self._launch(static_in, False)
                entry = (graph, static_in, out)
            except RuntimeError as e:
                warnings.warn(f"hifigan_b200: CUDA graph capture failed for shape {key}, running eagerly ({e})")
                torch.cuda.synchronize()
                entry = (None, None, None)
            if len(self.graphs) >= 8:
                self.graphs.pop(next(iter(self.graphs)))
            self.graphs[key] = entry
        graph, static_in, out = entry
        if graph is None:
            return self._launch(xin, False)
        static_in.copy_(xin)
        graph.replay()
        return out

    def _launch(self, xin: torch.Tensor, time_convs: bool, lengths: Optional[torch.Tensor] = None) -> torch.Tensor:
        L = _lib.lib()
        gen = self.gen
        b, c, frames = xin.shape
        ws = self.workspace(b, frames)
        nk = gen.num_kernels
        lp = 0 if lengths is None else lengths.data_ptr()
        mul = 1
        _lib.check(L.hg_ncl_to_nlc(xin.data_ptr(), b, c, frames, self.pre.cin_p, ws["mel"].data_ptr(), 0, 0.0,
                                   _stream()), "hg_ncl_to_nlc")
        if time_convs:
            ev0, ev1 = torch.cuda.Event(enable_timing=True), torch.cuda.Event(enable_timing=True)
            ev0.record()
        _conv(L, ws["mel"], self.pre, b, frames, out_act=ws["pre"], item=(lp, mul))
        cur, t = ws["pre"], frames
        for i, up in enumerate(self.ups):
            need_act = any(not _block_plan(L, gen.resblocks[i * nk + j], self.blocks[i * nk + j])[0]
                           for j in range(nk))
            _conv(L, cur, up, b, t, out_raw=ws["x_raw"], out_act=ws["x_act"] if need_act else None, item=(lp, mul))
            t *= up.stride
            mul *= up.stride
            c_p = up.cout_p
            last_stage = i == len(self.ups) - 1
            out_slope = 0.01 if last_stage else LRELU_SLOPE
            for j in range(nk):
                blk = gen.resblocks[i * nk + j]
                packs = self.blocks[i * nk + j]

                def final(kw, j=j):
                    if j < nk - 1:
                        others = (ws[f"r{j - 1}"] if (nk > 3 and j > 0) else None, None)
                        outs = dict(out_raw=ws[f"r{j}"])
                    else:
                        if nk > 3:
                            others = (ws[f"r{nk - 2}"], None)
                        else:
                            others = tuple(ws[f"r{q}"] for q in range(nk - 1)) + (None,) * (3 - nk)
                        outs = dict(scale=1.0 / nk, out_act=ws["stage_out"], slope=out_slope)
                    if "pair" in kw:
                        _pair(L, kw["x"], *kw["pair"], b, t, res=others, item=(lp, mul), **outs)
                    else:
                        _conv(L, kw["x"], kw["pc"], b, t, res=(kw["res0"],) + others, item=(lp, mul), **outs)

                _resblock_chain(L, blk, packs, b, t, c_p, ws["x_raw"], ws["x_act"], ws, final, item=(lp, mul))
            cur = ws["stage_out"]
        if time_convs:
            ev1.record()
            self.last_conv_events = (ev0, ev1)
        post = gen.conv_post
        _lib.check(L.hg_conv_post_tanh_fwd(cur.data_ptr(), self.post_w.data_ptr(), self.post_b.data_ptr(), b, t,
                                           self.post_cin_p, post.kernel_size[0], ws["y"].data_ptr(), _stream()),
                   "hg_conv_post_tanh_fwd")
        return ws["y"]


class Generator(torch.nn.Module):

    def __init__(self, h):
        super().__init__()
        self.h = h
        self.num_kernels = len(h.resblock_kernel_sizes)
        self.num_upsamples = len(h.upsample_rates)
        width = h.upsample_initial_channel
        self.conv_pre = _wn(Conv1d(80, width, 7, 1, padding=3))
        block_cls = ResBlock1 if h.resblock == '1' else ResBlock2

        self.ups = nn.ModuleList()
        for level, (rate, ksize) in enumerate(zip(h.upsample_rates, h.upsample_kernel_sizes)):
            self.ups.append(_wn(ConvTranspose1d(width >> level, width >> (level + 1), ksize, rate,
                                                padding=(ksize - rate) // 2)))
        self.resblocks = nn.ModuleList()
        for level in range(len(self.ups)):
            ch = width >> (level + 1)
            for ksize, dil in zip(h.resblock_kernel_sizes, h.resblock_dilation_sizes):
                self.resblocks.append(block_cls(h, ch, ksize, dil))
        self.conv_post = _wn(Conv1d(ch, 1, 7, 1, padding=3))
        self.ups.apply(init_weights)
        self.conv_post.apply(init_weights)
        self.__dict__["_hg_engines"] = {}

    def _engine(self, device) -> _GeneratorEngine:
        engines = self.__dict__.setdefault("_hg_engines", {})
        eng = engines.get(device)
        if eng is None:
            eng = _GeneratorEngine(self, device)
            engines[device] = eng
        return eng

    def forward(self, x: torch.Tensor, lengths: Optional[torch.Tensor] = None) -> torch.Tensor:
        _require_cuda(x, "Generator.forward")
        if x.dim() != 3 or x.shape[1] != self.conv_pre.in_channels:
            raise ValueError(f"expected [B,{self.conv_pre.in_channels},F], got {tuple(x.shape)}")
        if lengths is not None:
            if _wants_grad(x, self):
                raise NotImplementedError("ragged batches are an inference feature: call under torch.no_grad()")
            ln = torch.as_tensor(lengths).to(device=x.device, dtype=torch.int32).contiguous()
            if ln.shape != (x.shape[0],) or int(ln.min()) < 1 or int(ln.max()) > x.shape[2]:
                raise ValueError("lengths must be [B] frame counts within [1, F]")
            mask = torch.arange(x.shape[2], device=x.device)[None, None, :] < ln[:, None, None]
            return self._engine(x.device).forward(x * mask, lengths=ln).clone()
        if _wants_grad(x, self):
            from . import autograd
            return autograd.generator_forward(self, x)
        return self._engine(x.device).forward(x).clone()

    def _drop_engines(self):
        self.__dict__["_hg_engines"] = {}
        self.__dict__.pop("_hg_autograd", None)

    def remove_weight_norm(self):
        print('Removing weight norm...')
        for m in self.ups:
            remove_weight_norm(m)
        for blk in self.resblocks:
            blk.remove_weight_norm()
        remove_weight_norm(self.conv_pre)
        remove_weight_norm(self.conv_post)
        self._drop_engines()

    def _apply(self, fn, *args, **kwargs):
        out = super()._apply(fn, *args, **kwargs)
        self._drop_engines()
        return out


def _round_up(n: int, m: int) -> int:
    return (n + m - 1) // m * m


class _DiscLayer:

    def __init__(self, cin, cout, k, stride, pad, groups):
        self.cin, self.cout, self.k, self.stride, self.pad = cin, cout, k, stride, pad
        cin_g, cout_g = cin // groups, cout // groups
        merge = 1
        if groups == 1:
            if cin % 32 or cout % 32:
                raise NotImplementedError(f"conv {cin}->{cout}: channel counts must be multiples of 32")
        else:
            while (cin_g * merge) % 32 or (cout_g * merge) not in (32, 64, 128, 256):
                merge *= 2
                if merge > groups:
                    raise NotImplementedError(f"cannot tile conv {cin}->{cout} groups={groups}")
        self.groups, self.merge = groups, merge
        self.groups_eff = groups // merge
        self.cin_tile = cin if groups == 1 else cin_g * merge
        order = (c_int * k)()
        _lib.check(_lib.lib().hg_conv1d_tap_order(k, stride, pad, order), "hg_conv1d_tap_order")
        self.order = list(order)

    def pack(self, w: torch.Tensor) -> torch.Tensor:
        out = torch.empty(self.k, self.cout, self.cin_tile, dtype=torch.bfloat16, device=w.device)
        _lib.check(_lib.lib().hg_pack_disc_weight(w.data_ptr(), self.cout, self.cin, self.groups, self.merge, self.k,
                                                  self.stride, self.pad, out.data_ptr(), 0, _stream()),
                   "hg_pack_disc_weight")
        return out


class _SubDiscriminator(torch.nn.Module):

    def forward(self, x):
        _require_cuda(x, f"{type(self).__name__}.forward")
        from . import autograd
        return autograd.disc_forward(self, x, _wants_grad(x, self))


class DiscriminatorP(_SubDiscriminator):
    def __init__(self, period, kernel_size=5, stride=3, use_spectral_norm=False):
        super().__init__()
        self.period = period
        norm_f = spectral_norm if use_spectral_norm else _wn
        widths = [1, 32, 128, 512, 1024]
        layers = [norm_f(Conv2d(ci, co, (kernel_size, 1), (stride, 1), padding=(get_padding(5, 1), 0)))
                  for ci, co in zip(widths[:-1], widths[1:])]
        layers.append(norm_f(Conv2d(1024, 1024, (kernel_size, 1), 1, padding=(2, 0))))
        self.convs = nn.ModuleList(layers)
        self.conv_post = norm_f(Conv2d(1024, 1, (3, 1), 1, padding=(1, 0)))


class MultiPeriodDiscriminator(torch.nn.Module):
    def __init__(self):
        super().__init__()
        self.discriminators = nn.ModuleList([DiscriminatorP(p) for p in (2, 3, 5, 7, 11)])

    def forward(self, y, y_hat):
        y_d_rs, y_d_gs, fmap_rs, fmap_gs = [], [], [], []
        for d in self.discriminators:
            y_d_r, fmap_r = d(y)
            y_d_g, fmap_g = d(y_hat)
            y_d_rs.append(y_d_r); fmap_rs.append(fmap_r)
            y_d_gs.append(y_d_g); fmap_gs.append(fmap_g)
        return y_d_rs, y_d_gs, fmap_rs, fmap_gs


class DiscriminatorS(_SubDiscriminator):
    _SPEC = [(1, 128, 15, 1, 1, 7), (128, 128, 41, 2, 4, 20), (128, 256, 41, 2, 16, 20),
             (256, 512, 41, 4, 16, 20), (512, 1024, 41, 4, 16, 20), (1024, 1024, 41, 1, 16, 20),
             (1024, 1024, 5, 1, 1, 2)]

    def __init__(self, use_spectral_norm=False):
        super().__init__()
        norm_f = spectral_norm if use_spectral_norm else _wn
        self.convs = nn.ModuleList([norm_f(Conv1d(ci, co, k, s, groups=g, padding=p))
                                    for ci, co, k, s, g, p in self._SPEC])
        self.conv_post = norm_f(Conv1d(1024, 1, 3, 1, padding=1))

    def forward(self, x):
        out, fmap = super().forward(x)
        return out, [f.squeeze(-1) for f in fmap]


def _avgpool(x: torch.Tensor) -> torch.Tensor:
    t = x.shape[-1]
    xin = x.detach().reshape(-1, t).contiguous().float()
    out = torch.empty(*x.shape[:-1], t // 2 + 1, dtype=torch.float32, device=x.device)
    _lib.check(_lib.lib().hg_avgpool_4_2_2_fwd(xin.data_ptr(), xin.shape[0], t, out.data_ptr(), _stream()),
               "hg_avgpool_4_2_2_fwd")
    return out


class MultiScaleDiscriminator(torch.nn.Module):
    def __init__(self):
        super().__init__()
        self.discriminators = nn.ModuleList([DiscriminatorS(use_spectral_norm=True), DiscriminatorS(),
                                             DiscriminatorS()])
        self.meanpools = nn.ModuleList([AvgPool1d(4, 2, padding=2), AvgPool1d(4, 2, padding=2)])

    @staticmethod
    def _pool(x: torch.Tensor) -> torch.Tensor:
        if torch.is_grad_enabled() and x.requires_grad:
            from . import autograd
            return autograd.avgpool(x)
        return _avgpool(x)

    def forward(self, y, y_hat):
        _require_cuda(y, "MultiScaleDiscriminator.forward")
        _require_cuda(y_hat, "MultiScaleDiscriminator.forward")
        y_d_rs, y_d_gs, fmap_rs, fmap_gs = [], [], [], []
        for i, d in enumerate(self.discriminators):
            if i != 0:
                y, y_hat = self._pool(y), self._pool(y_hat)
            y_d_r, fmap_r = d(y)
            y_d_g, fmap_g = d(y_hat)
            y_d_rs.append(y_d_r); fmap_rs.append(fmap_r)
            y_d_gs.append(y_d_g); fmap_gs.append(fmap_g)
        return y_d_rs, y_d_gs, fmap_rs, fmap_gs


def _loss_mean(a32: torch.Tensor, b32: Optional[torch.Tensor], mode: int, c: float) -> torch.Tensor:
    acc = torch.zeros(1, dtype=torch.float32, device=a32.device)
    _lib.check(_lib.lib().hg_loss_sum(a32.data_ptr(), 0 if b32 is None else b32.data_ptr(), a32.numel(), mode, c,
                                      acc.data_ptr(), _stream()), "hg_loss_sum")
    return acc[0] / a32.numel()


def _device_mean(a: torch.Tensor, b: Optional[torch.Tensor], mode: int, c: float) -> torch.Tensor:
    if not a.is_cuda or (b is not None and not b.is_cuda):
        raise RuntimeError("hifigan_b200 losses have no CPU path; move the tensors to a B200")
    if torch.is_grad_enabled() and (a.requires_grad or (b is not None and b.requires_grad)):
        from . import autograd
        return autograd.device_mean(a, b, mode, c)
    return _loss_mean(a.detach().contiguous().float(), None if b is None else b.detach().contiguous().float(), mode, c)


def feature_loss(fmap_r, fmap_g):
    total = 0
    for maps_r, maps_g in zip(fmap_r, fmap_g):
        for r, g in zip(maps_r, maps_g):
            total = total + _device_mean(r, g, 0, 0.0)
    return total * 2


def discriminator_loss(disc_real_outputs, disc_generated_outputs):
    total, parts = 0, []
    for dr, dg in zip(disc_real_outputs, disc_generated_outputs):
        r_loss = _device_mean(dr, None, 1, 1.0)
        g_loss = _device_mean(dg, None, 1, 0.0)
        total = total + (r_loss + g_loss)
        parts += [r_loss.detach(), g_loss.detach()]
    host = torch.stack(parts).tolist() if parts else []
    return total, host[0::2], host[1::2]


def generator_loss(disc_outputs):
    gen_losses = [_device_mean(dg, None, 1, 1.0) for dg in disc_outputs]
    total = 0
    for l in gen_losses:
        total = total + l
    return total, gen_losses
```

include/hifigan_b200.h:

```cpp
#ifndef HIFIGAN_B200_H
#define HIFIGAN_B200_H

#include <stdint.h>

#ifdef __cplusplus
extern "C" {
#endif

#define HG_ABI_VERSION 3

const char* hg_version(void);
const char* hg_last_error(void);
int hg_abi_version(void);
int64_t hg_launch_count(void);
int hg_timestamp(uint64_t* dst, void* stream);

int hg_pack_conv1d_weight(const float* v, const float* g, int cout, int cin, int k, int cin_pad,
                          void* w_packed, void* stream);

int hg_convtr1d_geometry(int k, int stride, int padding, int* host_nshift, int* host_shift_min);

int hg_pack_convtr1d_weight(const float* v, const float* g, int cin, int cout, int k, int stride,
                            int padding, void* w_packed, void* stream);

int hg_conv1d_fwd(const void* x, const void* w_packed, const float* bias, int batch, int t, int cin,
                  int cout, int ktaps, int dilation, int pad_left, const void* res0,
                  const void* res1, const void* res2, float scale, void* out_raw, void* out_act,
                  float act_slope, const int* item_len, int item_mul, void* stream);

int hg_conv1d_tap_order(int ktaps, int stride, int pad_left, int* host_order);
int hg_conv1d_general_fwd(const void* x, const void* w_packed, const float* bias, int batch, int t_in_rows,
                          int c_total, int t_out, int t_out_rows, int groups, int cout, int ktaps, int stride,
                          int pad_left,
                          void* out_act, float act_slope, void* out_raw, int seq_pitch, int seq_valid, void* stream);

int hg_resblock_pair_supported(int c, int ktaps, int dil1);
int hg_resblock_single_supported(int c, int ktaps, int dil1);
int hg_resblock_pair_fwd(const void* x, const void* w1_packed, const float* b1, const void* w2_packed,
                         const float* b2, int batch, int t, int c, int ktaps, int dil1, float in_slope,
                         const void* res1, const void* res2, float scale, void* out_raw, void* out_act,
                         float out_slope, const int* item_len, int item_mul, void* stream);

int hg_disc_first_conv_fwd(const float* y, const float* w, const float* bias, int batch, int t, int period,
                           int k, int stride, int pad, int cout, int h_rows_out, void* out, float slope,
                           void* stream);
int hg_disc_last_conv_fwd(const void* x, const float* w, const float* bias, int nseq, int h, int h_rows, int c,
                          int k, float* out, void* stream);
int hg_avgpool_4_2_2_fwd(const float* x, int batch, int t, float* out, void* stream);
int hg_disc_export_fmap(const void* x, int batch, int period, int h, int h_rows, int c, float* out,
                        void* stream);
int hg_disc_import_fmap(const float* in, int batch, int period, int h, int h_rows, int c, void* x, void* stream);

int hg_ncl_to_nlc(const float* x, int batch, int c, int t, int c_pad, void* out, void* out_act,
                  float act_slope, void* stream);
int hg_nlc_to_ncl(const void* x, int batch, int t, int c, float* out, void* stream);

int hg_float_to_int16(const float* x, long long n, float scale, int16_t* out, void* stream);

int hg_loss_sum(const float* a, const float* b, long long n, int mode, float c, float* out_acc, void* stream);

int hg_segment_gather(const float* pool, const long long* start, const int* valid, int batch, int seg,
                      float* out, void* stream);

int hg_conv_post_tanh_fwd(const void* x, const float* w, const float* bias, int batch, int t, int c,
                          int k, float* y, void* stream);

typedef struct hg_mel_plan hg_mel_plan;
int hg_mel_plan_create(hg_mel_plan** out_plan, int n_fft, int num_mels, int sampling_rate,
                       int hop_size, int win_size, double fmin, double fmax ,
                       void* stream);
int hg_mel_plan_destroy(hg_mel_plan* plan);
int hg_mel_num_frames(const hg_mel_plan* plan, int t);
int hg_mel_fwd(const hg_mel_plan* plan, const float* y, int batch, int t, float* out,
               float* minmax, void* stream);

int hg_mel_bwd(const hg_mel_plan* plan, const float* y, const float* dmel, int batch, int t, float* dy,
               void* stream);

int hg_mel_bwd_emulate_host(const hg_mel_plan* plan, const float* host_y, const float* host_dmel, int batch, int t,
                            float* host_dy);

int hg_mel_emulate_host(const hg_mel_plan* plan, const float* host_y, int batch, int t,
                        float* host_out);


int hg_pack_dgrad_weight(const void* w_packed, int ktaps, int n, int c, void* out, void* stream);

int hg_conv1d_dgrad(const void* dy, const void* w_packed, int batch, int t_dy_valid, int t_dy_rows, int c_dy_total,
                    int t_out, int t_out_rows, int groups, int n_tile, int cout, int ktaps, int dilation, int pad_left,
                    const void* mask_src, float mask_slope, const void* fm_r, const void* fm_g, float fm_coef,
                    const void* res0, const void* res1, const void* res2, float scale, void* out, int seq_pitch,
                    int seq_valid, int seq_mul, int seq_div, const void* pre_add, float* bias_grad0,
                    float* bias_grad1, float* bias_grad2, int bias_mod, void* stream);

int hg_conv1d_wgrad(const void* x, const void* dy, int batch, int t_in_rows, int c_total, int t_out, int t_out_rows,
                    int groups, int cout, int ktaps, int stride, int dilation, int pad_left, float* dw_packed,
                    int accumulate, void* stream);

int hg_unpack_wgrad_conv(const float* dw_packed, int cout, int cin_g, int k, int rows_p, int cin_tile, int cout_g,
                         int merge, const int* host_tap_order, float* dw, void* stream);

int hg_wgrad_finish_conv(const float* dw_packed, int cout, int cin_g, int k, int rows_p, int cin_tile, int cout_g,
                         int merge, const int* host_tap_order, const float* v, const float* g, int accumulate,
                         float* dv, float* dg, void* stream);
int hg_wgrad_finish_convtr(const float* dw_packed, int cin, int cout, int k, int stride, int padding, int cin_p,
                           int cout_p, const float* v, const float* g, int accumulate, float* dv, float* dg,
                           void* stream);

int hg_weight_norm_bwd(const float* dw, const float* v, const float* g, int dim0, int rest, int accumulate,
                       float* dv, float* dg, void* stream);

int hg_fold_weight_norm(const float* v, const float* g, int dim0, int rest, float* w_eff, void* stream);
int hg_pack_disc_weight(const float* w_eff, int cout, int cin, int groups, int merge, int k, int stride, int pad,
                        void* w_fwd, void* w_dgrad, void* stream);

int hg_spectral_norm_fwd(const float* w, float* u, float* v, int rows, int cols, int iterate, float* w_eff,
                         float* sigma_out, float* u_copy, float* v_copy, float* ws, void* stream);
int hg_spectral_norm_bwd(const float* dw_eff, const float* w_eff, const float* u, const float* v, const float* sigma,
                         int rows, int cols, int accumulate, float* dw_orig, float* ws, void* stream);
enum {
  HG_JOB_GEN_CONV = 0, HG_JOB_GEN_CONVTR = 1, HG_JOB_GEN_POST = 2, HG_JOB_DISC_ROW = 3, HG_JOB_TRANSPOSE_TILE = 4,
  HG_JOB_DISC_DGRAD_TILE = 5, HG_JOB_FINISH_ROW = 6, HG_JOB_LOSS_SUM = 7
};
typedef struct hg_prep_job {
  const void* src0;
  const void* src1;
  const void* src2;
  void* dst0;
  void* dst1;
  int32_t kind;
  int32_t i[16];
  int32_t tab[64];
  int32_t pad_;
} hg_prep_job;
int hg_prep_job_size(void);
int hg_prep_batched(const hg_prep_job* jobs, const int* block_job, int first_block, int nblocks, int smem_bytes,
                    void* stream);

int hg_colsum_bf16(const void* x, int batch, int t_valid, int t_rows, int c, int accumulate, float* out, void* stream);

int hg_conv_post_tanh_bwd(const void* x, const float* w, const float* y, const float* dy, int batch, int t, int c,
                          int k, float in_slope, float dx_scale, void* dx, float* dpre_ws, float* dw, float* db,
                          float* bias_grad0, float* bias_grad1, float* bias_grad2, void* stream);

int hg_disc_last_conv_bwd(const void* x, const float* w, const float* dlogit, int nseq, int h, int h_rows, int c,
                          int k, float slope, const void* fm_r, float fm_coef, const void* pre_add, void* dx, float* dw,
                          float* db, float* bias_grad_in, void* stream);
int hg_disc_first_conv_bwd(const float* y, const float* w, const void* dpre, int batch, int t, int period, int k,
                           int stride, int pad, int cout, int h_rows, float* dw, float* db, float* dy, void* stream);
int hg_avgpool_4_2_2_bwd(const float* dout, int batch, int t, float* din, void* stream);

int hg_loss_grad(const float* a, const float* b, long long n, int mode, float c, float coef, float coef2,
                 const float* scale_dev, float* out, void* stream);

int hg_adamw_step(float* p, const float* g, float* m, float* v, long long n, float lr, float beta1, float beta2,
                  float eps, float weight_decay, int step, const int* dev_step, const float* dev_lr, float grad_scale,
                  void* stream);

#ifdef __cplusplus
}
#endif
#endif
```

Measured before the change: 333.5 million.

## Store only one activation form between resblock stages and invert leaky-ReLU for residuals

Resblock chain steps now write either the raw or the leaky-ReLU-activated tensor, not both. A consumer that needs the other form recovers the raw residual by inverting the leaky ReLU (min(x, x/slope)), either in the conv epilogue or in the fused pair kernel, which also skips its in-smem activation pass when handed activated input. This cuts one bf16 write per stage and the separate activation transform. The cost is an extra inversion in the epilogue and a slight precision change, because raw values are rebuilt from rounded activations.

```diff
diff --git a/hifi-gan_b200/_lib.py b/hifi-gan_b200/_lib.py
--- a/hifi-gan_b200/_lib.py
+++ b/hifi-gan_b200/_lib.py
@@ -105,6 +105,9 @@
     "hg_conv1d_fwd": (c_int, [c_void_p, c_void_p, c_void_p, c_int, c_int, c_int, c_int, c_int, c_int, c_int,
                               c_void_p, c_void_p, c_void_p, c_float, c_void_p, c_void_p, c_float, c_void_p, c_int,
                               c_void_p]),
+    "hg_conv1d_fwd_actres": (c_int, [c_void_p, c_void_p, c_void_p, c_int, c_int, c_int, c_int, c_int, c_int, c_int,
+                                     c_void_p, c_float, c_void_p, c_void_p, c_float, c_void_p, c_void_p, c_float,
+                                     c_void_p, c_int, c_void_p]),
     "hg_conv1d_tap_order": (c_int, [c_int, c_int, c_int, POINTER(c_int)]),
     "hg_conv1d_general_fwd": (c_int, [c_void_p, c_void_p, c_void_p, c_int, c_int, c_int, c_int, c_int, c_int, c_int,
                                       c_int, c_int, c_int, c_void_p, c_float, c_void_p, c_int, c_int, c_void_p]),
@@ -122,6 +125,9 @@
     "hg_resblock_pair_fwd": (c_int, [c_void_p, c_void_p, c_void_p, c_void_p, c_void_p, c_int, c_int, c_int, c_int,
                                      c_int, c_float, c_void_p, c_void_p, c_float, c_void_p, c_void_p, c_float,
                                      c_void_p, c_int, c_void_p]),
+    "hg_resblock_pair_fwd_actin": (c_int, [c_void_p, c_void_p, c_void_p, c_void_p, c_void_p, c_int, c_int, c_int,
+                                           c_int, c_int, c_float, c_void_p, c_void_p, c_float, c_void_p, c_void_p,
+                                           c_float, c_void_p, c_int, c_void_p]),
     "hg_float_to_int16": (c_int, [c_void_p, ctypes.c_longlong, c_float, c_void_p, c_void_p]),
     "hg_loss_sum": (c_int, [c_void_p, c_void_p, ctypes.c_longlong, c_int, c_float, c_void_p, c_void_p]),
     "hg_segment_gather": (c_int, [c_void_p, c_void_p, c_void_p, c_int, c_int, c_void_p, c_void_p]),
diff --git a/hifi-gan_b200/csrc/hg_common.cuh b/hifi-gan_b200/csrc/hg_common.cuh
--- a/hifi-gan_b200/csrc/hg_common.cuh
+++ b/hifi-gan_b200/csrc/hg_common.cuh
@@ -271,6 +271,14 @@
     v[2 * i + 1] += f.y;
   }
 }
+__device__ __forceinline__ void add_bf16x16_unlrelu(float (&v)[16], const U8& r, float inv_slope) {
+#pragma unroll
+  for (int i = 0; i < 8; ++i) {
+    const float2 f = unpack_bf16x2(r.v[i]);
+    v[2 * i] += fminf(f.x, f.x * inv_slope);
+    v[2 * i + 1] += fminf(f.y, f.y * inv_slope);
+  }
+}
 
 
 
diff --git a/hifi-gan_b200/csrc/hg_conv1d_tc.cu b/hifi-gan_b200/csrc/hg_conv1d_tc.cu
--- a/hifi-gan_b200/csrc/hg_conv1d_tc.cu
+++ b/hifi-gan_b200/csrc/hg_conv1d_tc.cu
@@ -54,6 +54,7 @@
   int colsum_mod;
   const int* item_len;
   int item_mul;
+  float res0_inv;
 };
 
 __host__ __device__ constexpr bool epi_mask(int k) { return k >= 2; }
@@ -61,6 +62,7 @@
 __host__ __device__ constexpr bool epi_fm(int k) { return k == 3 || k == 4; }
 __host__ __device__ constexpr bool epi_pre(int k) { return k == 4; }
 __host__ __device__ constexpr bool epi_mrf(int k) { return k >= 2; }
+__host__ __device__ constexpr bool epi_actres(int k) { return k == 0 || k == 5; }
 template <int kEpi>
 __device__ __forceinline__ void epi_group(const ConvArgs& p, bool valid, bool keep, size_t off, int ch,
                                           const uint32_t (&raw)[16], const hg::U8* r0, const hg::U8* r1,
@@ -98,7 +100,10 @@
       if (!(a.y > 0.f)) v[2 * i + 1] *= p.mask_slope;
     }
   }
-  if (p.res0) hg::add_bf16x16(v, *r0);
+  if (p.res0) {
+    if (epi_actres(kEpi)) hg::add_bf16x16_unlrelu(v, *r0, p.res0_inv);
+    else hg::add_bf16x16(v, *r0);
+  }
   if (epi_mrf(kEpi) && p.res1) hg::add_bf16x16(v, r1 ? *r1 : hg::ldg256(p.res1 + off));
   if (epi_mrf(kEpi) && p.res2) hg::add_bf16x16(v, r2 ? *r2 : hg::ldg256(p.res2 + off));
   const float sc = keep ? p.scale : 0.f;
@@ -786,6 +791,7 @@
   int colsum_mod = 0;
   const int* item_len = nullptr;
   int item_mul = 1;
+  float res0_inv = 1.f;
 };
 
 int conv_forward(const void* x, const void* w_packed, const float* bias, int batch, int t_in_rows,
@@ -892,6 +898,7 @@
   for (int i = 0; i < 3; ++i) p.colsum[i] = ex.colsum[i];
   p.colsum_mod = ex.colsum_mod > 0 ? ex.colsum_mod : cout;
   p.item_len = ex.item_len; p.item_mul = ex.item_mul;
+  p.res0_inv = ex.res0_inv;
   HG_REQUIRE(!ex.colsum[1] || ex.colsum[0], "conv: bias-gradient destinations must be filled from slot 0");
   p.seq_div = ex.seq_div > 0 ? ex.seq_div : (1 << 30);
   HG_REQUIRE(ex.seq_pitch >= 0 && (ex.seq_pitch == 0 || batch == 1), "conv: flat sequences need batch == 1");
@@ -944,11 +951,12 @@
 
 }
 
-extern "C" int hg_conv1d_fwd(const void* x, const void* w_packed, const float* bias, int batch, int t,
-                             int cin, int cout, int ktaps, int dilation, int pad_left,
-                             const void* res0, const void* res1, const void* res2, float scale,
-                             void* out_raw, void* out_act, float act_slope, const int* item_len, int item_mul,
-                             void* stream) {
+namespace {
+
+int conv1d_fwd(const void* x, const void* w_packed, const float* bias, int batch, int t, int cin, int cout, int ktaps,
+               int dilation, int pad_left, const void* res0, float res0_inv, const void* res1, const void* res2,
+               float scale, void* out_raw, void* out_act, float act_slope, const int* item_len, int item_mul,
+               void* stream) {
   HG_REQUIRE(cout > 0 && cout % 32 == 0, "hg_conv1d_fwd: cout=%d must be a multiple of 32", cout);
   HG_REQUIRE(cin > 0 && cin % 32 == 0, "hg_conv1d_fwd: cin=%d must be a multiple of 32", cin);
   HG_REQUIRE(ktaps > 0 && dilation > 0 && 128 + (ktaps - 1) * dilation <= 256,
@@ -956,8 +964,31 @@
   const int n_tile = (cout % 256 == 0) ? 256 : (cout % 128 == 0) ? 128 : (cout % 64 == 0) ? 64 : 32;
   ConvExtra ex;
   ex.item_len = item_len; ex.item_mul = item_mul > 0 ? item_mul : 1;
+  ex.res0_inv = res0_inv;
   return conv_forward(x, w_packed, bias, batch, t, cin, t, t, cin, cout, n_tile, 0, ktaps, 1, dilation, pad_left,
                       res0, res1, res2, scale, out_raw, out_act, act_slope, stream, ex);
+}
+
+}
+
+extern "C" int hg_conv1d_fwd(const void* x, const void* w_packed, const float* bias, int batch, int t,
+                             int cin, int cout, int ktaps, int dilation, int pad_left,
+                             const void* res0, const void* res1, const void* res2, float scale,
+                             void* out_raw, void* out_act, float act_slope, const int* item_len, int item_mul,
+                             void* stream) {
+  return conv1d_fwd(x, w_packed, bias, batch, t, cin, cout, ktaps, dilation, pad_left, res0, 1.f, res1, res2, scale,
+                    out_raw, out_act, act_slope, item_len, item_mul, stream);
+}
+
+extern "C" int hg_conv1d_fwd_actres(const void* x, const void* w_packed, const float* bias, int batch, int t,
+                                    int cin, int cout, int ktaps, int dilation, int pad_left,
+                                    const void* res0, float res0_slope, const void* res1, const void* res2,
+                                    float scale, void* out_raw, void* out_act, float act_slope, const int* item_len,
+                                    int item_mul, void* stream) {
+  HG_REQUIRE(res0 && res0_slope > 0.f && res0_slope <= 1.f,
+             "hg_conv1d_fwd_actres: needs res0 and a slope in (0, 1] (got %g)", res0_slope);
+  return conv1d_fwd(x, w_packed, bias, batch, t, cin, cout, ktaps, dilation, pad_left, res0, 1.f / res0_slope, res1,
+                    res2, scale, out_raw, out_act, act_slope, item_len, item_mul, stream);
 }
 
 extern "C" int hg_conv1d_tap_order(int ktaps, int stride, int pad_left, int* host_order) {
diff --git a/hifi-gan_b200/csrc/hg_resblock_pair.cu b/hifi-gan_b200/csrc/hg_resblock_pair.cu
--- a/hifi-gan_b200/csrc/hg_resblock_pair.cu
+++ b/hifi-gan_b200/csrc/hg_resblock_pair.cu
@@ -36,6 +36,7 @@
   __nv_bfloat16* out_act;
   const int* item_len;
   int item_mul;
+  float x_inv;
 };
 
 struct PairBarriers {
@@ -54,7 +55,7 @@
   return *reinterpret_cast<uint32_t*>(&v);
 }
 
-template <int C, bool kSingle, bool kMrf>
+template <int C, bool kSingle, bool kMrf, bool kActIn>
 __global__ void __launch_bounds__(pair_threads(C), 1)
 resblock_pair_kernel(const __grid_constant__ CUtensorMap tm_x, const __grid_constant__ CUtensorMap tm_w1,
                      const __grid_constant__ CUtensorMap tm_w2, const PairArgs p) {
@@ -211,14 +212,16 @@
     uint32_t slot = 0, phase = 0;
     for (int i = 0; i < n_local; ++i) {
       hg::mbar_wait(&bars->x_full[slot], phase);
-      uint4* xs = reinterpret_cast<uint4*>(x_buf + slot * p.x_slot_bytes);
-      for (int q = tid; q < n_chunks; q += kXformWarps * 32) {
-        uint4 v = xs[q];
-        v.x = lrelu_bf16x2(v.x, slope2); v.y = lrelu_bf16x2(v.y, slope2);
-        v.z = lrelu_bf16x2(v.z, slope2); v.w = lrelu_bf16x2(v.w, slope2);
-        xs[q] = v;
-      }
-      hg::fence_proxy_async_smem();
+      if (!kActIn) {
+        uint4* xs = reinterpret_cast<uint4*>(x_buf + slot * p.x_slot_bytes);
+        for (int q = tid; q < n_chunks; q += kXformWarps * 32) {
+          uint4 v = xs[q];
+          v.x = lrelu_bf16x2(v.x, slope2); v.y = lrelu_bf16x2(v.y, slope2);
+          v.z = lrelu_bf16x2(v.z, slope2); v.w = lrelu_bf16x2(v.w, slope2);
+          xs[q] = v;
+        }
+        hg::fence_proxy_async_smem();
+      }
       __syncwarp();
       if (lane == 0) hg::mbar_arrive(&bars->x_ready[slot]);
       if (++slot == static_cast<uint32_t>(p.x_slots)) { slot = 0; phase ^= 1u; }
@@ -359,7 +362,8 @@
               v[4 * q + 2] = __uint_as_float(raw[4 * q + 2]) + bq.z;
               v[4 * q + 3] = __uint_as_float(raw[4 * q + 3]) + bq.w;
             }
-            hg::add_bf16x16(v, rcur[g]);
+            if (kActIn) hg::add_bf16x16_unlrelu(v, rcur[g], p.x_inv);
+            else hg::add_bf16x16(v, rcur[g]);
             if (kMrf && p.res1) hg::add_bf16x16(v, kPreRes ? r1[kPreRes ? g : 0] : hg::ldg256(p.res1 + off + g * 16));
             if (kMrf && p.res2) hg::add_bf16x16(v, kPreRes ? r2[kPreRes ? g : 0] : hg::ldg256(p.res2 + off + g * 16));
             if (kMrf) {
@@ -395,24 +399,27 @@
 
 int g_sms = 0, g_smem = 0;
 
-template <int C, bool kSingle, bool kMrf>
+template <int C, bool kSingle, bool kMrf, bool kActIn>
 int launch_pair_as(const CUtensorMap& tx, const CUtensorMap& tw1, const CUtensorMap& tw2, const PairArgs& p,
                 size_t smem_bytes, int grid, cudaStream_t st) {
   static hg::PerDeviceOnce once;
   if (once.need())
-    HG_CHECK_CUDA(cudaFuncSetAttribute(resblock_pair_kernel<C, kSingle, kMrf>,
+    HG_CHECK_CUDA(cudaFuncSetAttribute(resblock_pair_kernel<C, kSingle, kMrf, kActIn>,
                                        cudaFuncAttributeMaxDynamicSharedMemorySize, g_smem));
-  resblock_pair_kernel<C, kSingle, kMrf><<<grid, pair_threads(C), smem_bytes, st>>>(tx, tw1, tw2, p);
+  resblock_pair_kernel<C, kSingle, kMrf, kActIn><<<grid, pair_threads(C), smem_bytes, st>>>(tx, tw1, tw2, p);
   HG_CHECK_CUDA(cudaGetLastError());
   return HG_OK;
 }
 
 template <int C, bool kSingle>
 int launch_pair(const CUtensorMap& tx, const CUtensorMap& tw1, const CUtensorMap& tw2, const PairArgs& p,
-                size_t smem_bytes, int grid, cudaStream_t st) {
+                bool act_in, size_t smem_bytes, int grid, cudaStream_t st) {
   const bool mrf = p.res1 || p.res2 || p.out_act || p.item_len || p.scale != 1.f;
-  return mrf ? launch_pair_as<C, kSingle, true>(tx, tw1, tw2, p, smem_bytes, grid, st)
-             : launch_pair_as<C, kSingle, false>(tx, tw1, tw2, p, smem_bytes, grid, st);
+  if (act_in)
+    return mrf ? launch_pair_as<C, kSingle, true, true>(tx, tw1, tw2, p, smem_bytes, grid, st)
+               : launch_pair_as<C, kSingle, false, true>(tx, tw1, tw2, p, smem_bytes, grid, st);
+  return mrf ? launch_pair_as<C, kSingle, true, false>(tx, tw1, tw2, p, smem_bytes, grid, st)
+             : launch_pair_as<C, kSingle, false, false>(tx, tw1, tw2, p, smem_bytes, grid, st);
 }
 
 size_t pair_smem_bytes(int c, int ktaps, int dil1, int subs, int x_slots, int single, PairArgs* out) {
@@ -458,11 +465,12 @@
   return pick_subs(c, ktaps, dil1, 1) > 0 ? 1 : 0;
 }
 
-extern "C" int hg_resblock_pair_fwd(const void* x, const void* w1_packed, const float* b1,
-                                    const void* w2_packed, const float* b2, int batch, int t, int c,
-                                    int ktaps, int dil1, float in_slope, const void* res1,
-                                    const void* res2, float scale, void* out_raw, void* out_act,
-                                    float out_slope, const int* item_len, int item_mul, void* stream) {
+namespace {
+
+int resblock_pair_fwd(const void* x, bool act_in, const void* w1_packed, const float* b1, const void* w2_packed,
+                      const float* b2, int batch, int t, int c, int ktaps, int dil1, float in_slope, const void* res1,
+                      const void* res2, float scale, void* out_raw, void* out_act, float out_slope,
+                      const int* item_len, int item_mul, void* stream) {
   const int single = w2_packed == nullptr;
   HG_REQUIRE(x && w1_packed && b1 && (single || b2), "hg_resblock_pair_fwd: null input");
   HG_REQUIRE(out_raw || out_act, "hg_resblock_pair_fwd: no output requested");
@@ -490,6 +498,7 @@
   p.out_raw = static_cast<__nv_bfloat16*>(out_raw);
   p.out_act = static_cast<__nv_bfloat16*>(out_act);
   p.item_len = item_len; p.item_mul = item_mul > 0 ? item_mul : 1;
+  p.x_inv = act_in ? 1.f / in_slope : 1.f;
 
   CUtensorMap tx, tw1, tw2;
   const int swz = c * 2;
@@ -505,12 +514,33 @@
   const int grid = p.num_tiles < g_sms ? p.num_tiles : g_sms;
   cudaStream_t st = static_cast<cudaStream_t>(stream);
   if (single)
-    rc = (c == 64) ? launch_pair<64, true>(tx, tw1, tw2, p, smem_bytes, grid, st)
-                   : launch_pair<32, true>(tx, tw1, tw2, p, smem_bytes, grid, st);
+    rc = (c == 64) ? launch_pair<64, true>(tx, tw1, tw2, p, act_in, smem_bytes, grid, st)
+                   : launch_pair<32, true>(tx, tw1, tw2, p, act_in, smem_bytes, grid, st);
   else
-    rc = (c == 64) ? launch_pair<64, false>(tx, tw1, tw2, p, smem_bytes, grid, st)
-                   : launch_pair<32, false>(tx, tw1, tw2, p, smem_bytes, grid, st);
+    rc = (c == 64) ? launch_pair<64, false>(tx, tw1, tw2, p, act_in, smem_bytes, grid, st)
+                   : launch_pair<32, false>(tx, tw1, tw2, p, act_in, smem_bytes, grid, st);
   if (rc) return rc;
   g_hg_launches.fetch_add(1, std::memory_order_relaxed);
   return HG_OK;
 }
+
+}
+
+extern "C" int hg_resblock_pair_fwd(const void* x, const void* w1_packed, const float* b1,
+                                    const void* w2_packed, const float* b2, int batch, int t, int c,
+                                    int ktaps, int dil1, float in_slope, const void* res1,
+                                    const void* res2, float scale, void* out_raw, void* out_act,
+                                    float out_slope, const int* item_len, int item_mul, void* stream) {
+  return resblock_pair_fwd(x, false, w1_packed, b1, w2_packed, b2, batch, t, c, ktaps, dil1, in_slope, res1, res2,
+                           scale, out_raw, out_act, out_slope, item_len, item_mul, stream);
+}
+
+extern "C" int hg_resblock_pair_fwd_actin(const void* x_act, const void* w1_packed, const float* b1,
+                                          const void* w2_packed, const float* b2, int batch, int t, int c,
+                                          int ktaps, int dil1, float in_slope, const void* res1,
+                                          const void* res2, float scale, void* out_raw, void* out_act,
+                                          float out_slope, const int* item_len, int item_mul, void* stream) {
+  HG_REQUIRE(in_slope > 0.f && in_slope <= 1.f, "hg_resblock_pair_fwd_actin: slope %g not in (0, 1]", in_slope);
+  return resblock_pair_fwd(x_act, true, w1_packed, b1, w2_packed, b2, batch, t, c, ktaps, dil1, in_slope, res1, res2,
+                           scale, out_raw, out_act, out_slope, item_len, item_mul, stream);
+}
diff --git a/hifi-gan_b200/models.py b/hifi-gan_b200/models.py
--- a/hifi-gan_b200/models.py
+++ b/hifi-gan_b200/models.py
@@ -149,25 +149,28 @@
         self.key = key
 
 
-def _conv(L, x, pc: _PackedConv, batch: int, t: int, *, res=(None, None, None), scale=1.0,
+def _conv(L, x, pc: _PackedConv, batch: int, t: int, *, res=(None, None, None), res0_slope=0.0, scale=1.0,
           out_raw=None, out_act=None, slope=LRELU_SLOPE, item=(0, 1)) -> None:
     p = [0 if r is None else r.data_ptr() for r in res]
-    _lib.check(L.hg_conv1d_fwd(x.data_ptr(), pc.w.data_ptr(), pc.bias.data_ptr(), batch, t, pc.cin_p,
-                               pc.w.shape[1], pc.taps, pc.dil, pc.pad_left, p[0], p[1], p[2], scale,
-                               0 if out_raw is None else out_raw.data_ptr(),
-                               0 if out_act is None else out_act.data_ptr(), slope, item[0], item[1], _stream()),
-               "hg_conv1d_fwd")
-
-
-def _pair(L, x, pc1: _PackedConv, pc2: _PackedConv, batch: int, t: int, *, res=(None, None), scale=1.0,
-          out_raw=None, out_act=None, slope=LRELU_SLOPE, item=(0, 1)) -> None:
+    outs = (0 if out_raw is None else out_raw.data_ptr(), 0 if out_act is None else out_act.data_ptr(), slope,
+            item[0], item[1], _stream())
+    head = (x.data_ptr(), pc.w.data_ptr(), pc.bias.data_ptr(), batch, t, pc.cin_p, pc.w.shape[1], pc.taps, pc.dil,
+            pc.pad_left)
+    if res0_slope:
+        _lib.check(L.hg_conv1d_fwd_actres(*head, p[0], res0_slope, p[1], p[2], scale, *outs), "hg_conv1d_fwd_actres")
+    else:
+        _lib.check(L.hg_conv1d_fwd(*head, p[0], p[1], p[2], scale, *outs), "hg_conv1d_fwd")
+
+
+def _pair(L, x, pc1: _PackedConv, pc2: _PackedConv, batch: int, t: int, *, x_act=False, res=(None, None),
+          scale=1.0, out_raw=None, out_act=None, slope=LRELU_SLOPE, item=(0, 1)) -> None:
     p = [0 if r is None else r.data_ptr() for r in res]
     w2, b2 = (0, 0) if pc2 is None else (pc2.w.data_ptr(), pc2.bias.data_ptr())
-    _lib.check(L.hg_resblock_pair_fwd(x.data_ptr(), pc1.w.data_ptr(), pc1.bias.data_ptr(), w2,
-                                      b2, batch, t, pc1.cin_p, pc1.taps, pc1.dil, LRELU_SLOPE,
-                                      p[0], p[1], scale, 0 if out_raw is None else out_raw.data_ptr(),
-                                      0 if out_act is None else out_act.data_ptr(), slope, item[0], item[1], _stream()),
-               "hg_resblock_pair_fwd")
+    fn, name = ((L.hg_resblock_pair_fwd_actin, "hg_resblock_pair_fwd_actin") if x_act
+                else (L.hg_resblock_pair_fwd, "hg_resblock_pair_fwd"))
+    _lib.check(fn(x.data_ptr(), pc1.w.data_ptr(), pc1.bias.data_ptr(), w2, b2, batch, t, pc1.cin_p, pc1.taps,
+                  pc1.dil, LRELU_SLOPE, p[0], p[1], scale, 0 if out_raw is None else out_raw.data_ptr(),
+                  0 if out_act is None else out_act.data_ptr(), slope, item[0], item[1], _stream()), name)
 
 
 _FUSE_PAIRS = True
@@ -198,24 +201,27 @@
     for i in range(steps):
         last = i == steps - 1
         nr, na = ping[i & 1]
-        want_act = (not last) and (not fused[i + 1])
+        if not last:
+            nr, na = (nr, None) if fused[i + 1] else (None, na)
         if fused[i]:
             pc1, pc2 = (packs[2 * i], packs[2 * i + 1]) if two_conv else (packs[i], None)
+            x, x_is_act = (cur_raw, False) if cur_raw is not None else (cur_act, True)
             if last:
-                final(dict(pair=(pc1, pc2), x=cur_raw))
+                final(dict(pair=(pc1, pc2), x=x, x_act=x_is_act))
             else:
-                _pair(L, cur_raw, pc1, pc2, batch, t, out_raw=nr, out_act=na if want_act else None, item=item)
+                _pair(L, x, pc1, pc2, batch, t, x_act=x_is_act, out_raw=nr, out_act=na, item=item)
         else:
             if two_conv:
                 _conv(L, cur_act, packs[2 * i], batch, t, out_act=bufs["t1"], item=item)
                 src, pc = bufs["t1"], packs[2 * i + 1]
             else:
                 src, pc = cur_act, packs[i]
+            res0, res0_slope = (cur_raw, 0.0) if cur_raw is not None else (cur_act, LRELU_SLOPE)
             if last:
-                final(dict(pc=pc, x=src, res0=cur_raw))
+                final(dict(pc=pc, x=src, res0=res0, res0_slope=res0_slope))
             else:
-                _conv(L, src, pc, batch, t, res=(cur_raw, None, None), out_raw=nr,
-                      out_act=na if (want_act or not two_conv) else None, item=item)
+                _conv(L, src, pc, batch, t, res=(res0, None, None), res0_slope=res0_slope, out_raw=nr, out_act=na,
+                      item=item)
         cur_raw, cur_act = nr, na
 
 
@@ -248,9 +254,10 @@
 
         def final(kw):
             if "pair" in kw:
-                _pair(L, kw["x"], *kw["pair"], b, t, out_raw=bufs["out"])
+                _pair(L, kw["x"], *kw["pair"], b, t, x_act=kw["x_act"], out_raw=bufs["out"])
             else:
-                _conv(L, kw["x"], kw["pc"], b, t, res=(kw["res0"], None, None), out_raw=bufs["out"])
+                _conv(L, kw["x"], kw["pc"], b, t, res=(kw["res0"], None, None), res0_slope=kw["res0_slope"],
+                      out_raw=bufs["out"])
 
         _resblock_chain(L, self, packs, b, t, c_p, bufs["x_raw"], bufs["x_act"], bufs, final)
         y = torch.empty(b, c_p, t, dtype=torch.float32, device=x.device)
@@ -463,7 +470,8 @@
         for i, up in enumerate(self.ups):
             need_act = any(not _block_plan(L, gen.resblocks[i * nk + j], self.blocks[i * nk + j])[0]
                            for j in range(nk))
-            _conv(L, cur, up, b, t, out_raw=ws["x_raw"], out_act=ws["x_act"] if need_act else None, item=(lp, mul))
+            x_raw, x_act = (None, ws["x_act"]) if need_act else (ws["x_raw"], None)
+            _conv(L, cur, up, b, t, out_raw=x_raw, out_act=x_act, item=(lp, mul))
             t *= up.stride
             mul *= up.stride
             c_p = up.cout_p
@@ -484,11 +492,12 @@
                             others = tuple(ws[f"r{q}"] for q in range(nk - 1)) + (None,) * (3 - nk)
                         outs = dict(scale=1.0 / nk, out_act=ws["stage_out"], slope=out_slope)
                     if "pair" in kw:
-                        _pair(L, kw["x"], *kw["pair"], b, t, res=others, item=(lp, mul), **outs)
+                        _pair(L, kw["x"], *kw["pair"], b, t, x_act=kw["x_act"], res=others, item=(lp, mul), **outs)
                     else:
-                        _conv(L, kw["x"], kw["pc"], b, t, res=(kw["res0"],) + others, item=(lp, mul), **outs)
-
-                _resblock_chain(L, blk, packs, b, t, c_p, ws["x_raw"], ws["x_act"], ws, final, item=(lp, mul))
+                        _conv(L, kw["x"], kw["pc"], b, t, res=(kw["res0"],) + others, res0_slope=kw["res0_slope"],
+                              item=(lp, mul), **outs)
+
+                _resblock_chain(L, blk, packs, b, t, c_p, x_raw, x_act, ws, final, item=(lp, mul))
             cur = ws["stage_out"]
         if time_convs:
             ev1.record()
diff --git a/include/hifigan_b200.h b/include/hifigan_b200.h
--- a/include/hifigan_b200.h
+++ b/include/hifigan_b200.h
@@ -27,6 +27,10 @@
                   int cout, int ktaps, int dilation, int pad_left, const void* res0,
                   const void* res1, const void* res2, float scale, void* out_raw, void* out_act,
                   float act_slope, const int* item_len, int item_mul, void* stream);
+int hg_conv1d_fwd_actres(const void* x, const void* w_packed, const float* bias, int batch, int t, int cin,
+                         int cout, int ktaps, int dilation, int pad_left, const void* res0, float res0_slope,
+                         const void* res1, const void* res2, float scale, void* out_raw, void* out_act,
+                         float act_slope, const int* item_len, int item_mul, void* stream);
 
 int hg_conv1d_tap_order(int ktaps, int stride, int pad_left, int* host_order);
 int hg_conv1d_general_fwd(const void* x, const void* w_packed, const float* bias, int batch, int t_in_rows,
@@ -40,6 +44,10 @@
                          const float* b2, int batch, int t, int c, int ktaps, int dil1, float in_slope,
                          const void* res1, const void* res2, float scale, void* out_raw, void* out_act,
                          float out_slope, const int* item_len, int item_mul, void* stream);
+int hg_resblock_pair_fwd_actin(const void* x_act, const void* w1_packed, const float* b1, const void* w2_packed,
+                               const float* b2, int batch, int t, int c, int ktaps, int dil1, float in_slope,
+                               const void* res1, const void* res2, float scale, void* out_raw, void* out_act,
+                               float out_slope, const int* item_len, int item_mul, void* stream);
 
 int hg_disc_first_conv_fwd(const float* y, const float* w, const float* bias, int batch, int t, int period,
                            int k, int stride, int pad, int cout, int h_rows_out, void* out, float slope,
```

Result: faster. 347.9 million (median of 6 runs) (+4.3%).
